# davidsd/sdpb

Hardware: AMD Instinct MI355X
Metric: interior-point iterations/sec at --precision 512 (higher is better)
Workload: dtype mw576 (fixed-width multi-word float, 18x32-bit limbs; Q syrk: exact integer product of a fixed-point image with 509 fraction bits)

## Files before the change

sdpb_amd/csrc/kernels.hpp:

```cpp
#pragma once
#include "dev.hpp"
#include "mw_wave.hpp"
#include "tiledot.hpp"

#include <algorithm>
#include <cmath>
#include <cstdlib>

namespace sdpb
{
using mw::Mw;
using mw::Acc;
constexpr int WG = 256;

template <int NL> MW_HD Mw<NL> mat_ld(const Batch &b, const MatDesc &d, int i, int j)
{
  return mw::load<NL>(b.p, (size_t)d.off + (size_t)i + (size_t)j * (size_t)d.ld);
}
template <int NL> MW_HD void mat_st(const Batch &b, const MatDesc &d, int i, int j, const Mw<NL> &v)
{
  mw::store<NL>(b.p, (size_t)d.off + (size_t)i + (size_t)j * (size_t)d.ld, v);
}

template <int NL, int STRIDE> MW_HD Mw<NL> smem_ld(const uint32_t *s, int idx)
// ... 1380 lines not shown
__global__ void __launch_bounds__(WG) k_dual_residues(Batch AY, mw::CPtr c, mw::Ptr d, const BlockDesc *blk)
{
  const int j = blockIdx.y;
  const BlockDesc bl = blk[j];
  const int p = blockIdx.x * WG + threadIdx.x;
  if(p >= bl.P)
    return;
  int cb, rb, k;
  decode_p(p, bl.K, cb, rb, k);
  Mw<NL> acc = mw::load<NL>(c, (size_t)bl.voff + p);
  for(int b = 0; b < 2; ++b)
    {
      const MatDesc dy = AY.d[2 * j + b];
      acc = mw::sub(acc, mat_ld<NL>(AY, dy, cb * bl.K + k, rb * bl.K + k));
    }
  mw::store<NL>(d, (size_t)bl.voff + p, acc);
}

template <int NL> __global__ void __launch_bounds__(WG) k_scale_bases(Batch bases, mw::CPtr a, Batch scaled, const BlockDesc *blk)
{
  const int q = blockIdx.y;
  const BlockDesc bl = blk[q >> 1];
  const MatDesc dbs = bases.d[q], dsc = scaled.d[q];
  const int rs = bl.rows[q & 1], K = bl.K;
  const int idx = blockIdx.x * WG + threadIdx.x;
  if(idx >= dsc.rows * dsc.cols)
    return;
  const int k = idx % K, col = idx / K, pair = col / rs, jj = col % rs;
  mat_st<NL>(scaled, dsc, k, col, mw::mul(mat_ld<NL>(bases, dbs, jj, k), mw::load<NL>(a, (size_t)bl.voff + (size_t)pair * K + k)));
}
template <int NL>
__global__ void __launch_bounds__(WG) k_constraint_weighted_sum(Batch bases, Batch scaled, Batch out, Batch addend,
                                                                int addend_sign, const BlockDesc *blk)
{
  const int q = blockIdx.y;
  const BlockDesc bl = blk[q >> 1];
  const MatDesc dout = out.d[q], dbs = bases.d[q], dsc = scaled.d[q];
  const int n = dout.rows, rs = bl.rows[q & 1];
  const int idx = blockIdx.x * WG + threadIdx.x;
  if(idx >= n * n)
    return;
  const int I = idx % n, Jc = idx / n;
  const int bi = I / rs, i = I % rs, bj = Jc / rs, jj = Jc % rs;
  const int hi = bi > bj ? bi : bj, lo = bi > bj ? bj : bi;
  const int col = (hi * (hi + 1) / 2 + lo) * rs + jj;
  Acc<NL> sum = mw::acc_zero<NL>();
  for(int k = 0; k < bl.K; ++k)
    mw::acc_fma(sum, mat_ld<NL>(bases, dbs, i, k), mat_ld<NL>(scaled, dsc, k, col));
  Mw<NL> acc = mw::acc_result(sum);
  if(hi != lo)
    acc = mw::mul_2exp(acc, -1);
  if(addend_sign)
    {
      const Mw<NL> ad = mat_ld<NL>(addend, addend.d[q], I, Jc);
      acc = addend_sign > 0 ? mw::add(acc, ad) : mw::sub(acc, ad);
    }
  mat_st<NL>(out, dout, I, Jc, acc);
}

template <int NL>
__global__ void __launch_bounds__(WG)
  k_schur_rhs2(Batch basesT, Batch Z, mw::CPtr dres, mw::Ptr dx, const BlockDesc *blk)
{
  const int j = blockIdx.y, t = threadIdx.x;
  const BlockDesc bl = blk[j];
  const int pair = blockIdx.x;
  if(pair >= bl.m * (bl.m + 1) / 2)
    return;
  int cb = 0;
  while((cb + 1) * (cb + 2) / 2 <= pair)
    ++cb;
  const int rb = pair - cb * (cb + 1) / 2;
  const int K = bl.K, KL = K < WG ? K : WG, G = WG / KL;
  const int kk = t % KL, g = t / KL;
  __shared__ Mw<NL> part[WG];
  for(int k0 = 0; k0 < K; k0 += KL)
    {
      const int k = k0 + kk;
      Acc<NL> colsum = mw::acc_zero<NL>();
      if(g < G && k < K)
        for(int b = 0; b < 2; ++b)
          {
            const int rs = bl.rows[b];
            const MatDesc dz = Z.d[2 * j + b], dbt = basesT.d[2 * j + b];
            for(int i = g; i < rs; i += G)
              {
                Acc<NL> zq = mw::acc_zero<NL>();
                for(int l = 0; l < rs; ++l)
                  mw::acc_fma(zq, mat_ld<NL>(Z, dz, cb * rs + l, rb * rs + i), mat_ld<NL>(basesT, dbt, k, l));
                mw::acc_fma(colsum, mw::acc_result(zq), mat_ld<NL>(basesT, dbt, k, i));
              }
          }
      part[t] = mw::acc_result(colsum);
      __syncthreads();
      if(g == 0 && k < K)
        {
          const size_t p = (size_t)bl.voff + (size_t)pair * K + k;
          Acc<NL> sum = mw::acc_zero<NL>();
          mw::acc_add(sum, mw::load<NL>(dres, p), 1u);
          for(int gg = 0; gg < G; ++gg)
            mw::acc_add(sum, part[gg * KL + kk], 1u);
          mw::store<NL>(dx, p, mw::acc_result(sum));
        }
      __syncthreads();
    }
}

template <int NL, bool TRANS>
__global__ void __launch_bounds__(WG) k_vec_trsm(Batch L, Batch Li, Batch X)
{
  const int q = blockIdx.x, t = threadIdx.x;
  const MatDesc dl = L.d[q], di = Li.d[q], dx = X.d[q];
  const int n = dl.rows;
  if(n == 0)
    return;
  constexpr int SEG = WG / PB;
  const int i = t % PB, seg = t / PB;
  const int panels = (n + PB - 1) / PB;
  __shared__ Mw<NL> sx[PB], part[WG];
  auto vec = [&](int r) { return (size_t)dx.off + (size_t)r * dx.ld; };
  for(int pp = 0; pp < panels; ++pp)
    {
      const int p = TRANS ? panels - 1 - pp : pp;
      const int k0 = p * PB, nb = n - k0 < PB ? n - k0 : PB;
      Acc<NL> acc = mw::acc_zero<NL>();
      if(i < nb)
        {
          const int lo = TRANS ? k0 + nb : 0, hi = TRANS ? n : k0;
          for(int k = lo + seg; k < hi; k += SEG)
            {
              const Mw<NL> l = TRANS ? mat_ld<NL>(L, dl, k, k0 + i) : mat_ld<NL>(L, dl, k0 + i, k);
              mw::acc_fms(acc, l, mw::load<NL>(X.p, vec(k)));
            }
          if(seg == 0)
            mw::acc_add(acc, mw::load<NL>(X.p, vec(k0 + i)));
        }
      part[t] = mw::acc_result(acc);
      __syncthreads();
      if(t < nb)
        {
          Acc<NL> s = mw::acc_zero<NL>();
          for(int gsg = 0; gsg < SEG; ++gsg)
            mw::acc_add(s, part[gsg * PB + t]);
          sx[t] = mw::acc_result(s);
        }
      __syncthreads();
      acc = mw::acc_zero<NL>();
      if(i < nb)
        for(int k = seg; k < nb; k += SEG)
          if(TRANS ? k >= i : k <= i)
            mw::acc_fma(acc, TRANS ? mat_ld<NL>(Li, di, k0 + k, k0 + i) : mat_ld<NL>(Li, di, k0 + i, k0 + k), sx[k]);
      part[t] = mw::acc_result(acc);
      __syncthreads();
      if(t < nb)
        {
          Acc<NL> s = mw::acc_zero<NL>();
          for(int gsg = 0; gsg < SEG; ++gsg)
            mw::acc_add(s, part[gsg * PB + t]);
          mw::store<NL>(X.p, vec(k0 + t), mw::acc_result(s));
        }
      __syncthreads();
    }
}

template <int NL, bool SQUARE>
__global__ void __launch_bounds__(WG) k_gemv_t_partial(Batch MT, mw::CPtr v, mw::Ptr part, const BlockDesc *blk, int N)
{
  const int j = blockIdx.y;
  const BlockDesc bl = blk[j];
  const int n = blockIdx.x * WG + threadIdx.x;
  if(n >= N)
    return;
  const MatDesc dm = MT.d[j];
  Acc<NL> acc = mw::acc_zero<NL>();
  for(int p = 0; p < bl.P; ++p)
    {
      const Mw<NL> a = mat_ld<NL>(MT, dm, n, p);
      if(SQUARE)
        mw::acc_fma(acc, a, a);
      else
        mw::acc_fma(acc, a, mw::load<NL>(v, (size_t)bl.voff + p));
    }
  mw::store<NL>(part, (size_t)j * N + n, mw::acc_result(acc));
}
template <int NL>
__global__ void __launch_bounds__(WG) k_sum_partials(mw::CPtr part, int J, int N, mw::CPtr base, int has_base, int sign, mw::Ptr out)
{
  constexpr int SP_G = 8, SP_N = WG / SP_G;
  const int i = threadIdx.x % SP_N, g = threadIdx.x / SP_N;
  const int n = blockIdx.x * SP_N + i;
  __shared__ Mw<NL> sm[WG];
  Acc<NL> acc = mw::acc_zero<NL>();
  if(n < N)
    for(int j = g; j < J; j += SP_G)
      mw::acc_add(acc, mw::load<NL>(part, (size_t)j * N + n), sign < 0 ? 1u : 0u);
  sm[threadIdx.x] = mw::acc_result(acc);
  __syncthreads();
  if(g != 0 || n >= N)
    return;
  Acc<NL> tot = mw::acc_zero<NL>();
  for(int gg = 0; gg < SP_G; ++gg)
    mw::acc_add(tot, sm[gg * SP_N + i]);
  if(has_base)
    mw::acc_add(tot, mw::load<NL>(base, n));
  mw::store<NL>(out, n, mw::acc_result(tot));
}
constexpr int SP_ROWS = WG / 8;
template <int NL>
__global__ void __launch_bounds__(WG) k_gemv_n(Batch MT, mw::CPtr v, mw::Ptr out, const BlockDesc *blk, int N, int sign)
{
  const int j = blockIdx.y;
  const BlockDesc bl = blk[j];
  const int lane = threadIdx.x & 63, sub = threadIdx.x >> 6;
  const int p = blockIdx.x * 4 + sub;
  Acc<NL> sum = mw::acc_zero<NL>();
  if(p < bl.P)
    {
      const MatDesc dm = MT.d[j];
      for(int n = lane; n < N; n += 64)
        mw::acc_fma(sum, mat_ld<NL>(MT, dm, n, p), mw::load<NL>(v, n));
    }
#if defined(__HIP_DEVICE_COMPILE__)
  {
    const Mw<NL> mine = mw::acc_result(sum);
    Acc<NL> a = mw::acc_zero<NL>();
    for(int g = 0; g < 8; ++g)
      mw::acc_add(a, wave_get<NL>(mine, g * 8 + (lane & 7)));
    const Mw<NL> s8 = mw::acc_result(a);
    Acc<NL> t = mw::acc_zero<NL>();
    if(p < bl.P)
      mw::acc_add(t, mw::load<NL>(out, (size_t)bl.voff + p));
    for(int g = 0; g < 8; ++g)
      mw::acc_add(t, wave_get<NL>(s8, g), sign < 0 ? 1u : 0u);
    if(lane == 0 && p < bl.P)
      mw::store<NL>(out, (size_t)bl.voff + p, mw::acc_result(t));
  }
#else
  __shared__ uint32_t sm[(NL + 2) * WG];
  smem_st<NL, WG>(sm, threadIdx.x, mw::acc_result(sum));
  __syncthreads();
  if(lane < 8)
    {
      Acc<NL> a = mw::acc_zero<NL>();
      for(int g = 0; g < 8; ++g)
        mw::acc_add(a, smem_ld<NL, WG>(sm, sub * 64 + g * 8 + lane));
      smem_st<NL, WG>(sm, threadIdx.x, mw::acc_result(a));
    }
  __syncthreads();
  if(lane == 0 && p < bl.P)
    {
      Acc<NL> a = mw::acc_zero<NL>();
      mw::acc_add(a, mw::load<NL>(out, (size_t)bl.voff + p));
      for(int g = 0; g < 8; ++g)
        mw::acc_add(a, smem_ld<NL, WG>(sm, sub * 64 + g), sign < 0 ? 1u : 0u);
      mw::store<NL>(out, (size_t)bl.voff + p, mw::acc_result(a));
    }
#endif
}

template <int FX> constexpr bool fx_two_level()
{
#ifdef SDPB_SYRK_ONE_LEVEL
  return false;
#else
  return FX % 4 == 0 && FX <= 32;
#endif
}
template <int NL> constexpr int fx_limbs() { return (NL - 2 >= 14 && (NL - 2) % 4 != 0) ? ((NL - 2 + 3) / 4) * 4 : NL - 2; }
#ifndef SDPB_TOOM4_MAX_FX
#define SDPB_TOOM4_MAX_FX 48
#endif
template <int FX> constexpr bool fx_toom4()
{
#if defined(SDPB_SYRK_ONE_LEVEL) || defined(SDPB_SYRK_NO_TOOM4)
  return false;
#else
  return FX % 4 == 0 && FX >= 16 && FX <= SDPB_TOOM4_MAX_FX;
#endif
}
template <int FX> constexpr bool fx_toom4k()
{
#if defined(SDPB_SYRK_NO_TOOM4K)
  return false;
#else
  return fx_toom4<FX>() && (FX == 16 || FX == 24 || FX == 32);
#endif
}
template <int FX> constexpr bool fx_toom5k()
{
#if defined(SDPB_SYRK_NO_TOOM5K)
  return false;
#else
  return fx_toom4k<FX>() && FX == 16;
#endif
}
constexpr int T5_LB = 28;
constexpr uint32_t T5_MASK = (1u << T5_LB) - 1u;
constexpr int T5_H = 55;
template <int FX> constexpr int fx_nprod() { return fx_toom5k<FX>() ? 27 : 21; }
template <int FX> constexpr int fx_part_limbs() { return fx_toom5k<FX>() ? 5 : 2 * (FX / 8) + 1; }
template <int FX> constexpr int toom_wb() { return fx_toom5k<FX>() ? 102 : 32 * (FX / 4) - (fx_toom4k<FX>() ? 6 : 4); }
template <int FX> constexpr int fx_planes()
{
  return fx_toom5k<FX>() ? 27 * 2 : fx_toom4k<FX>() ? 21 * (FX / 8) : fx_toom4<FX>() ? 7 * (FX / 4) : fx_two_level<FX>() ? 9 * (FX / 4) : 3 * (FX / 2);
}
template <int FX> constexpr int fx_frac_bits()
{
  return fx_toom5k<FX>() ? 5 * toom_wb<FX>() - 1 : fx_toom4<FX>() ? 4 * toom_wb<FX>() - 1 : fx_two_level<FX>() ? 32 * FX - 7 : 32 * FX - 3;
}
template <int FX> constexpr int fx_col_slot(int c) { return fx_toom5k<FX>() ? 32 * (c / 32) + 2 * (c % 16) + (c % 32) / 16 : c; }
template <int FX> constexpr size_t fx_row_slots(size_t cols) { return fx_toom5k<FX>() ? (cols + 31) / 32 * 32 : cols; }
template <int FX> MW_HD size_t fx_elem(size_t idx, int N)
{
  if constexpr(fx_toom5k<FX>())
    return idx / (size_t)N * fx_row_slots<FX>((size_t)N) + (size_t)fx_col_slot<FX>((int)(idx % (size_t)N));
  else
    return idx;
}
template <int FX> constexpr size_t fx_image_stride(size_t rows, size_t cols, int rb)
{
  return fx_toom4k<FX>() ? (rows + rb - 1) / rb * rb * fx_row_slots<FX>(cols) + 64 : rows * cols;
}
template <int FX> constexpr int syrk_tile_edge() { return fx_toom4k<FX>() ? 32 : 16; }

template <int BIT0, int NB, int W, int OUT> MW_HD void bits_slice(const uint32_t (&x)[W], uint32_t (&out)[OUT])
{
  constexpr int q = BIT0 / 32, r = BIT0 % 32;
#pragma unroll
  for(int i = 0; i < OUT; ++i)
    {
      const uint32_t lo = (q + i < W) ? x[q + i < W ? q + i : 0] : 0u;
      const uint32_t hi = (q + i + 1 < W) ? x[q + i + 1 < W ? q + i + 1 : 0] : 0u;
      uint32_t v = r ? ((lo >> r) | (hi << ((32 - r) & 31))) : lo;
      const int left = NB - 32 * i;
      if(left <= 0)
        v = 0;
      else if(left < 32)
        v &= (1u << (left & 31)) - 1u;
      out[i] = v;
    }
}

template <int W, int A> MW_HD void add_shifted(uint32_t (&w)[W], const uint32_t (&x)[A], int sh, bool negate)
{
  const int q = sh >> 5, r = sh & 31;
  uint64_t cy = negate ? 1u : 0u;
  const uint32_t mask = negate ? 0xffffffffu : 0u;
#pragma unroll
  for(int k = 0; k < W; ++k)
    {
      const int i0 = k - q;
      uint32_t lo = 0, hi = 0;
#pragma unroll
      for(int t = 0; t < A; ++t)
        {
          lo = (t == i0 - 1) ? x[t] : lo;
          hi = (t == i0) ? x[t] : hi;
        }
      const uint32_t limb = r ? ((hi << r) | (lo >> (32 - r))) : hi;
      const uint64_t s = (uint64_t)w[k] + (uint64_t)(limb ^ mask) + cy;
      w[k] = (uint32_t)s;
      cy = s >> 32;
    }
}

template <int FX> MW_HD void fx_store2(const uint32_t (&mag)[FX], bool negative, uint32_t *fx, size_t fx_stride, size_t idx);
template <int FX> MW_HD void fx_store4(const uint32_t (&mag)[FX], bool negative, uint32_t *fx, size_t fx_stride, size_t idx);
template <int FX> MW_HD void fx_store5(const uint32_t (&mag)[FX], bool negative, uint32_t *fx, size_t fx_stride, size_t idx);
template <int FX> MW_HD void fx_store(const uint32_t (&mag)[FX], bool negative, uint32_t *fx, size_t fx_stride, size_t idx)
{
  constexpr int M = FX / 2;
  static_assert(FX % 2 == 0 && FX >= 4, "FX = NL - 2 is even");
  if constexpr(fx_toom5k<FX>())
    {
      fx_store5<FX>(mag, negative, fx, fx_stride, idx);
      return;
    }
  else if constexpr(fx_toom4<FX>())
    {
      fx_store4<FX>(mag, negative, fx, fx_stride, idx);
      return;
    }
  else if constexpr(fx_two_level<FX>())
    {
      fx_store2<FX>(mag, negative, fx, fx_stride, idx);
      return;
    }
  uint32_t a[FX];
  uint64_t borrow = 0;
#pragma unroll
  for(int i = 0; i < FX; ++i)
    {
      const uint32_t c = (i == FX - 1) ? (1u << 29) : 0u;
      if(negative)
        {
          const uint64_t d = (uint64_t)c - (uint64_t)mag[i] - borrow;
          a[i] = (uint32_t)d;
          borrow = (d >> 63) & 1u;
        }
      else
        a[i] = mag[i] | c;
    }
  uint32_t lo[M], hi[M];
#pragma unroll
  for(int i = 0; i < M; ++i)
    {
      lo[i] = (i == M - 1) ? (a[i] & 0x7fffffffu) : a[i];
      const uint32_t up = (M + i < FX) ? a[M + i < FX ? M + i : 0] : 0u;
      hi[i] = (a[M - 1 + i] >> 31) | (up << 1);
    }
  uint64_t cy = 0;
#pragma unroll
  for(int i = 0; i < M; ++i)
    {
      const uint64_t s = (uint64_t)lo[i] + hi[i] + cy;
      cy = s >> 32;
      fx[(size_t)i * fx_stride + idx] = lo[i];
      fx[(size_t)(M + i) * fx_stride + idx] = hi[i];
      fx[(size_t)(2 * M + i) * fx_stride + idx] = (uint32_t)s;
    }
}

template <int FX> MW_HD void fx_store2(const uint32_t (&mag)[FX], bool negative, uint32_t *fx, size_t fx_stride, size_t idx)
{
  constexpr int M = FX / 2, M2 = FX / 4, FB = fx_frac_bits<FX>();
  static_assert(FB / 32 == FX - 1, "the bias bit sits in the top limb");
  uint32_t a[FX];
  uint64_t borrow = 0;
#pragma unroll
  for(int i = 0; i < FX; ++i)
    {
      const uint32_t c = (i == FX - 1) ? (1u << (FB % 32)) : 0u;
      if(negative)
        {
          const uint64_t d = (uint64_t)c - (uint64_t)mag[i] - borrow;
          a[i] = (uint32_t)d;
          borrow = (d >> 63) & 1u;
        }
      else
        a[i] = mag[i] | c;
    }
  uint32_t x[3][M];
  bits_slice<0, 32 * M - 3>(a, x[0]);
  bits_slice<32 * M - 3, 32 * M - 3>(a, x[1]);
  {
    uint64_t cy = 0;
#pragma unroll
    for(int i = 0; i < M; ++i)
      {
        const uint64_t t = (uint64_t)x[0][i] + x[1][i] + cy;
        x[2][i] = (uint32_t)t;
        cy = t >> 32;
      }
  }
#pragma unroll
  for(int k = 0; k < 3; ++k)
    {
      uint32_t p0[M2], p1[M2];
      bits_slice<0, 32 * M2 - 1>(x[k], p0);
      bits_slice<32 * M2 - 1, 32 * M2 - 1>(x[k], p1);
      uint32_t *o0 = fx + ((size_t)(3 * k) * fx_stride + idx) * M2, *o1 = fx + ((size_t)(3 * k + 1) * fx_stride + idx) * M2,
               *ot = fx + ((size_t)(3 * k + 2) * fx_stride + idx) * M2;
      uint64_t cy = 0;
#pragma unroll
      for(int i = 0; i < M2; ++i)
        {
          const uint64_t t = (uint64_t)p0[i] + p1[i] + cy;
          cy = t >> 32;
          o0[i] = p0[i];
          o1[i] = p1[i];
          ot[i] = (uint32_t)t;
        }
    }
}

struct alignas(16) PieceQuad
{
  uint32_t w[4];
};
struct alignas(8) PiecePair
{
  uint32_t w[2];
};
template <int M2> MW_HD void piece_load(const uint32_t *p, uint32_t (&x)[M2])
{
  if constexpr(M2 % 4 == 0)
    {
#pragma unroll
      for(int q = 0; q < M2 / 4; ++q)
        {
          const PieceQuad v = *reinterpret_cast<const PieceQuad *>(p + 4 * q);
#pragma unroll
          for(int l = 0; l < 4; ++l)
            x[4 * q + l] = v.w[l];
        }
    }
  else if constexpr(M2 % 2 == 0)
    {
#pragma unroll
      for(int q = 0; q < M2 / 2; ++q)
        {
          const PiecePair v = *reinterpret_cast<const PiecePair *>(p + 2 * q);
          x[2 * q] = v.w[0];
          x[2 * q + 1] = v.w[1];
        }
    }
  else
    {
#pragma unroll
      for(int l = 0; l < M2; ++l)
        x[l] = p[l];
    }
}
template <int M2> MW_HD void piece_store(uint32_t *p, const uint32_t (&x)[M2])
{
  if constexpr(M2 % 4 == 0)
    {
#pragma unroll
      for(int q = 0; q < M2 / 4; ++q)
        {
          PieceQuad v;
#pragma unroll
          for(int l = 0; l < 4; ++l)
            v.w[l] = x[4 * q + l];
          *reinterpret_cast<PieceQuad *>(p + 4 * q) = v;
        }
    }
  else if constexpr(M2 % 2 == 0)
    {
#pragma unroll
      for(int q = 0; q < M2 / 2; ++q)
        {
          PiecePair v;
          v.w[0] = x[2 * q];
          v.w[1] = x[2 * q + 1];
          *reinterpret_cast<PiecePair *>(p + 2 * q) = v;
        }
    }
  else
    {
#pragma unroll
      for(int l = 0; l < M2; ++l)
        p[l] = x[l];
    }
}

template <int A> MW_HD void sub_limbs(uint32_t (&d)[A], const uint32_t (&x)[A])
{
  uint64_t bw = 0;
#pragma unroll
  for(int k = 0; k < A; ++k)
    {
      const uint64_t t = (uint64_t)d[k] - (uint64_t)x[k] - bw;
      d[k] = (uint32_t)t;
      bw = (t >> 63) & 1u;
    }
}

template <int ML> MW_HD void toom5_lin(uint32_t (&out)[ML], const uint32_t (&p)[5][ML], uint32_t c0, uint32_t c1, uint32_t c2, uint32_t c3, uint32_t c4)
{
  uint64_t cy = 0;
#pragma unroll
  for(int i = 0; i < ML; ++i)
    {
      const uint64_t t = (uint64_t)p[0][i] * c0 + (uint64_t)p[1][i] * c1 + (uint64_t)p[2][i] * c2 + (uint64_t)p[3][i] * c3 + (uint64_t)p[4][i] * c4 + cy;
      out[i] = (uint32_t)t;
      cy = t >> 32;
    }
}
template <int POS, int NB, int ML> MW_HD uint32_t toom5_bits(const uint32_t (&x)[ML])
{
  constexpr int q = POS / 32, r = POS % 32;
  const uint32_t lo = q < ML ? x[q < ML ? q : 0] : 0u, hi = q + 1 < ML ? x[q + 1 < ML ? q + 1 : 0] : 0u;
  const uint32_t v = r ? ((lo >> r) | (hi << (32 - r))) : lo;
  return NB < 32 ? (v & ((1u << (NB < 32 ? NB : 0)) - 1u)) : v;
}
template <int FX> MW_HD void fx_store5(const uint32_t (&mag)[FX], bool negative, uint32_t *fx, size_t fx_stride, size_t idx)
{
  constexpr int WB = toom_wb<FX>(), FB = fx_frac_bits<FX>(), ML = (WB + 7 + 31) / 32, H = T5_H, LB = T5_LB;
  constexpr int TOPBIT = WB - 32 * (ML - 1);
  static_assert(FB == 5 * WB - 1 && FB / 32 == FX - 1, "a' = v + 2^FB fills five pieces of WB bits");
  static_assert(TOPBIT >= 0 && TOPBIT + 7 <= 32 && WB + 7 <= 2 * H && H + 1 <= 2 * LB, "121 b fits, the halves fit two limbs");
  uint32_t a[FX];
  uint64_t borrow = 0;
#pragma unroll
  for(int i = 0; i < FX; ++i)
    {
      const uint32_t c = (i == FX - 1) ? (1u << (FB % 32)) : 0u;
      if(negative)
        {
          const uint64_t d = (uint64_t)c - (uint64_t)mag[i] - borrow;
          a[i] = (uint32_t)d;
          borrow = (d >> 63) & 1u;
        }
      else
        a[i] = mag[i] | c;
    }
  uint32_t p[5][ML];
  bits_slice<0, WB>(a, p[0]);
  bits_slice<WB, WB>(a, p[1]);
  bits_slice<2 * WB, WB>(a, p[2]);
  bits_slice<3 * WB, WB>(a, p[3]);
  bits_slice<4 * WB, WB>(a, p[4]);
  uint32_t e[9][ML];
#pragma unroll
  for(int i = 0; i < ML; ++i)
    {
      e[0][i] = p[0][i];
      e[8][i] = p[4][i];
    }
  toom5_lin<ML>(e[1], p, 1, 1, 1, 1, 1);
  toom5_lin<ML>(e[3], p, 1, 2, 4, 8, 16);
  toom5_lin<ML>(e[5], p, 16, 8, 4, 2, 1);
  toom5_lin<ML>(e[7], p, 1, 3, 9, 27, 81);
  {
    uint32_t pos[ML], neg[ML];
    auto diff = [&](uint32_t (&out)[ML], uint32_t bias) {
      pos[ML - 1] += bias << TOPBIT;
      uint64_t bw = 0;
#pragma unroll
      for(int i = 0; i < ML; ++i)
        {
          const uint64_t t = (uint64_t)pos[i] - (uint64_t)neg[i] - bw;
          out[i] = (uint32_t)t;
          bw = (t >> 63) & 1u;
        }
    };
    toom5_lin<ML>(pos, p, 1, 0, 1, 0, 1);
    toom5_lin<ML>(neg, p, 0, 1, 0, 1, 0);
    diff(e[2], 2u);
    toom5_lin<ML>(pos, p, 1, 0, 4, 0, 16);
    toom5_lin<ML>(neg, p, 0, 2, 0, 8, 0);
    diff(e[4], 10u);
    toom5_lin<ML>(pos, p, 16, 0, 4, 0, 1);
    toom5_lin<ML>(neg, p, 0, 8, 0, 2, 0);
    diff(e[6], 10u);
  }
#pragma unroll
  for(int g = 0; g < 9; ++g)
    {
      uint32_t lo[2], hi[2], mid[2];
      lo[0] = toom5_bits<0, LB>(e[g]);
      lo[1] = toom5_bits<LB, H - LB>(e[g]);
      hi[0] = toom5_bits<H, LB>(e[g]);
      hi[1] = toom5_bits<H + LB, H - LB>(e[g]);
      const uint32_t s0 = lo[0] + hi[0];
      mid[0] = s0 & T5_MASK;
      mid[1] = lo[1] + hi[1] + (s0 >> LB);
      piece_store<2>(fx + ((size_t)(3 * g + 0) * fx_stride + idx) * 2, lo);
      piece_store<2>(fx + ((size_t)(3 * g + 1) * fx_stride + idx) * 2, hi);
      piece_store<2>(fx + ((size_t)(3 * g + 2) * fx_stride + idx) * 2, mid);
    }
}

template <int M2> MW_HD void toom_lin(uint32_t (&out)[M2], const uint32_t (&p)[4][M2], uint32_t c0, uint32_t c1, uint32_t c2, uint32_t c3)
{
  uint64_t cy = 0;
#pragma unroll
  for(int i = 0; i < M2; ++i)
    {
      const uint64_t t = (uint64_t)p[0][i] * c0 + (uint64_t)p[1][i] * c1 + (uint64_t)p[2][i] * c2 + (uint64_t)p[3][i] * c3 + cy;
      out[i] = (uint32_t)t;
      cy = t >> 32;
    }
}
template <int FX> MW_HD void fx_store4(const uint32_t (&mag)[FX], bool negative, uint32_t *fx, size_t fx_stride, size_t idx)
{
  constexpr int M2 = FX / 4, WB = toom_wb<FX>(), FB = fx_frac_bits<FX>();
  constexpr int TOPBIT = WB - 32 * (M2 - 1);
  static_assert(FB == 4 * WB - 1 && FB / 32 == FX - 1, "a' = v + 2^FB fills four pieces of WB bits");
  static_assert(TOPBIT >= 0 && TOPBIT + 4 <= 32, "15 b fits the top limb");
  uint32_t a[FX];
  uint64_t borrow = 0;
#pragma unroll
  for(int i = 0; i < FX; ++i)
    {
      const uint32_t c = (i == FX - 1) ? (1u << (FB % 32)) : 0u;
      if(negative)
        {
          const uint64_t d = (uint64_t)c - (uint64_t)mag[i] - borrow;
          a[i] = (uint32_t)d;
          borrow = (d >> 63) & 1u;
        }
      else
        a[i] = mag[i] | c;
    }
  uint32_t p[4][M2];
  bits_slice<0, WB>(a, p[0]);
  bits_slice<WB, WB>(a, p[1]);
  bits_slice<2 * WB, WB>(a, p[2]);
  bits_slice<3 * WB, WB>(a, p[3]);
  uint32_t e[7][M2];
#pragma unroll
  for(int i = 0; i < M2; ++i)
    {
      e[0][i] = p[0][i];
      e[6][i] = p[3][i];
    }
  toom_lin<M2>(e[1], p, 1, 1, 1, 1);
  toom_lin<M2>(e[3], p, 1, 2, 4, 8);
  toom_lin<M2>(e[5], p, 8, 4, 2, 1);
  {
    uint32_t pos[M2], neg[M2];
    toom_lin<M2>(pos, p, 1, 0, 1, 0);
    toom_lin<M2>(neg, p, 0, 1, 0, 1);
    pos[M2 - 1] += 2u << TOPBIT;
    uint64_t bw = 0;
#pragma unroll
    for(int i = 0; i < M2; ++i)
      {
        const uint64_t t = (uint64_t)pos[i] - (uint64_t)neg[i] - bw;
        e[2][i] = (uint32_t)t;
        bw = (t >> 63) & 1u;
      }
    toom_lin<M2>(pos, p, 1, 0, 4, 0);
    toom_lin<M2>(neg, p, 0, 2, 0, 8);
    pos[M2 - 1] += 10u << TOPBIT;
    bw = 0;
#pragma unroll
    for(int i = 0; i < M2; ++i)
      {
        const uint64_t t = (uint64_t)pos[i] - (uint64_t)neg[i] - bw;
        e[4][i] = (uint32_t)t;
        bw = (t >> 63) & 1u;
      }
  }
  if constexpr(fx_toom4k<FX>())
    {
      constexpr int M3 = FX / 8, H = 16 * M2 - 1;
#pragma unroll
      for(int g = 0; g < 7; ++g)
        {
          uint32_t lo[M3], hi[M3], mid[M3];
          bits_slice<0, H>(e[g], lo);
          bits_slice<H, H>(e[g], hi);
          uint64_t cy = 0;
#pragma unroll
          for(int i = 0; i < M3; ++i)
            {
              const uint64_t t = (uint64_t)lo[i] + hi[i] + cy;
              mid[i] = (uint32_t)t;
              cy = t >> 32;
            }
          piece_store<M3>(fx + ((size_t)(3 * g + 0) * fx_stride + idx) * M3, lo);
          piece_store<M3>(fx + ((size_t)(3 * g + 1) * fx_stride + idx) * M3, hi);
          piece_store<M3>(fx + ((size_t)(3 * g + 2) * fx_stride + idx) * M3, mid);
        }
    }
  else
    {
#pragma unroll
      for(int g = 0; g < 7; ++g)
        {
          uint32_t *o = fx + ((size_t)g * fx_stride + idx) * M2;
#pragma unroll
          for(int i = 0; i < M2; ++i)
            o[i] = e[g][i];
        }
    }
}
template <int FX> MW_HD void toom_piece_load(const uint32_t *fx, size_t fx_stride, int g, size_t e, uint32_t (&x)[FX / 4])
{
  constexpr int M2 = FX / 4;
  if constexpr(fx_toom4k<FX>())
    {
      constexpr int M3 = FX / 8, H = 16 * M2 - 1;
      uint32_t lo[M2], lo3[M3], hi[M3];
      piece_load<M3>(fx + ((size_t)(3 * g + 0) * fx_stride + e) * M3, lo3);
      piece_load<M3>(fx + ((size_t)(3 * g + 1) * fx_stride + e) * M3, hi);
#pragma unroll
      for(int i = 0; i < M2; ++i)
        lo[i] = i < M3 ? lo3[i < M3 ? i : 0] : 0u;
      add_shifted<M2, M3>(lo, hi, H, false);
#pragma unroll
      for(int i = 0; i < M2; ++i)
        x[i] = lo[i];
    }
  else
    {
      const uint32_t *src = fx + ((size_t)g * fx_stride + e) * M2;
#pragma unroll
      for(int i = 0; i < M2; ++i)
        x[i] = src[i];
    }
}
template <int Z> MW_HD void z_add(uint32_t (&d)[Z], const uint32_t (&x)[Z])
{
  uint64_t cy = 0;
#pragma unroll
  for(int k = 0; k < Z; ++k)
    {
      const uint64_t t = (uint64_t)d[k] + x[k] + cy;
      d[k] = (uint32_t)t;
      cy = t >> 32;
    }
}
template <int Z> MW_HD void z_sub(uint32_t (&d)[Z], const uint32_t (&x)[Z])
{
  uint64_t bw = 0;
#pragma unroll
  for(int k = 0; k < Z; ++k)
    {
      const uint64_t t = (uint64_t)d[k] - (uint64_t)x[k] - bw;
      d[k] = (uint32_t)t;
      bw = (t >> 63) & 1u;
    }
}
template <int Z> MW_HD void z_addmul(uint32_t (&d)[Z], const uint32_t (&x)[Z], uint32_t c, bool subtract)
{
  uint32_t t[Z];
  uint64_t cy = 0;
#pragma unroll
  for(int k = 0; k < Z; ++k)
    {
      const uint64_t u = (uint64_t)x[k] * c + cy;
      t[k] = (uint32_t)u;
      cy = u >> 32;
    }
  if(subtract)
    z_sub<Z>(d, t);
  else
    z_add<Z>(d, t);
}
template <int Z> MW_HD void z_sar(uint32_t (&d)[Z], int bits)
{
  const uint32_t fill = 0u - (d[Z - 1] >> 31);
#pragma unroll
  for(int k = 0; k < Z; ++k)
    {
      const uint32_t up = k + 1 < Z ? d[k + 1 < Z ? k + 1 : 0] : fill;
      d[k] = (d[k] >> bits) | (up << (32 - bits));
    }
}
template <int Z> MW_HD void z_shl(uint32_t (&d)[Z], int sh)
{
  const int q = sh >> 5, r = sh & 31;
  uint32_t t[Z];
#pragma unroll
  for(int k = 0; k < Z; ++k)
    {
      uint32_t lo = 0, hi = 0;
#pragma unroll
      for(int u = 0; u < Z; ++u)
        {
          hi = (u == k - q) ? d[u] : hi;
          lo = (u == k - q - 1) ? d[u] : lo;
        }
      t[k] = r ? ((hi << r) | (lo >> (32 - r))) : hi;
    }
#pragma unroll
  for(int k = 0; k < Z; ++k)
    d[k] = t[k];
}
template <int Z> MW_HD void z_divexact(uint32_t (&d)[Z], uint32_t c, uint32_t cinv)
{
  uint32_t carry = 0;
#pragma unroll
  for(int k = 0; k < Z; ++k)
    {
      const uint32_t b = d[k] < carry ? 1u : 0u;
      const uint32_t q = (d[k] - carry) * cinv;
      d[k] = q;
      carry = (uint32_t)(((uint64_t)q * c) >> 32) + b;
    }
}
template <int Z> MW_HD void toom4_interpolate(uint32_t (&w)[7][Z])
{
  z_add<Z>(w[5], w[4]);
  {
    uint32_t t[Z];
#pragma unroll
    for(int k = 0; k < Z; ++k)
      t[k] = w[4][k];
    z_sub<Z>(t, w[1]);
    z_sar<Z>(t, 1);
#pragma unroll
    for(int k = 0; k < Z; ++k)
      w[1][k] = t[k];
  }
  z_sub<Z>(w[4], w[0]);
  z_sub<Z>(w[4], w[1]);
  z_sar<Z>(w[4], 2);
  z_addmul<Z>(w[4], w[6], 16, true);
  {
    uint32_t t[Z];
#pragma unroll
    for(int k = 0; k < Z; ++k)
      t[k] = w[2][k];
    z_sub<Z>(t, w[3]);
    z_sar<Z>(t, 1);
#pragma unroll
    for(int k = 0; k < Z; ++k)
      w[3][k] = t[k];
  }
  z_sub<Z>(w[2], w[3]);
  z_addmul<Z>(w[5], w[2], 65, true);
  z_sub<Z>(w[2], w[6]);
  z_sub<Z>(w[2], w[0]);
  z_addmul<Z>(w[5], w[2], 45, false);
  z_sar<Z>(w[5], 1);
  z_sub<Z>(w[4], w[2]);
  z_divexact<Z>(w[4], 3, 0xAAAAAAABu);
  z_sub<Z>(w[2], w[4]);
  {
    uint32_t t[Z];
#pragma unroll
    for(int k = 0; k < Z; ++k)
      t[k] = w[5][k];
    z_sub<Z>(t, w[1]);
#pragma unroll
    for(int k = 0; k < Z; ++k)
      w[1][k] = t[k];
  }
  z_addmul<Z>(w[5], w[3], 8, true);
  z_divexact<Z>(w[5], 9, 0x38E38E39u);
  z_sub<Z>(w[3], w[5]);
  z_divexact<Z>(w[1], 15, 0xEEEEEEEFu);
  z_add<Z>(w[1], w[5]);
  z_sar<Z>(w[1], 1);
  z_sub<Z>(w[5], w[1]);
}

template <int NL, int FX>
__global__ void __launch_bounds__(WG) k_normalize_fx(mw::CPtr PT, size_t count, int N, mw::CPtr inv_norm, uint32_t *fx, size_t fx_stride)
{
  constexpr int FB = fx_frac_bits<FX>();
  for(size_t idx = (size_t)blockIdx.x * WG + threadIdx.x; idx < count; idx += (size_t)gridDim.x * WG)
    {
      const Mw<NL> t = mw::mul(mw::load<NL>(PT, idx), mw::load<NL>(inv_norm, idx % N));
      uint32_t w[NL];
      bool sat = false;
      if(mw::is_zero(t))
        {
#pragma unroll
          for(int i = 0; i < NL; ++i)
            w[i] = 0;
        }
      else
        {
#pragma unroll
          for(int i = 0; i < NL; ++i)
            w[i] = t.m[i];
          const int s = 32 * NL - FB - t.e;
          if(t.e >= 1)
            sat = true;
          else if(s >= 32 * NL)
            {
#pragma unroll
              for(int i = 0; i < NL; ++i)
                w[i] = 0;
            }
          else
            {
              mw::shr_limbs<NL>(w, (uint32_t)s >> 5);
// ... 548 lines not shown
  {
    uint32_t m[Z];
#pragma unroll
    for(int k = 0; k < Z; ++k)
      m[k] = 0;
    z_addmul<Z>(m, t, 10, false);
    z_shl<Z>(m, WB);
#pragma unroll
    for(int k = 0; k < Z; ++k)
      t[k] = 0;
    z_addmul<Z>(t, n, 50, false);
    z_shl<Z>(t, 2 * WB);
    z_add<Z>(t, m);
  }
#pragma unroll
  for(int k = 0; k < Z; ++k)
    toomU[(size_t)(Z + k) * N + col] = t[k];
}
template <int FX>
__global__ void __launch_bounds__(WG)
  k_syrk4_finish(const uint32_t *part, int nsplit, size_t part_stride, const uint32_t *tile_list, size_t total, const uint32_t *toomU,
                 uint32_t *acc, size_t acc_stride, int N, int col0, int col1)
{
  constexpr int M2 = FX / 4, A2 = 2 * M2 + 1, Z = 2 * M2 + 2, W = 2 * FX + 2, WB = toom_wb<FX>();
  const size_t pidx = (size_t)blockIdx.x * WG + threadIdx.x;
  int i, j;
  if(pidx >= total || !syrk_packed_decode<syrk_tile_edge<FX>()>(pidx, tile_list, N, col0, col1, i, j))
    return;
  const size_t idx = (size_t)i + (size_t)j * N;
  uint32_t w[7][Z];
  constexpr int GRP[7] = {0, 4, 1, 2, 3, 5, 6};
  if constexpr(fx_toom4k<FX>())
    {
      constexpr int M3 = FX / 8, A3 = 2 * M3 + 1, H = 16 * M2 - 1;
#pragma unroll
      for(int q = 0; q < 7; ++q)
        {
          uint32_t g3[3][A3];
#pragma unroll
          for(int u = 0; u < 3; ++u)
            {
              uint64_t cy = 0;
#pragma unroll
              for(int k = 0; k < A3; ++k)
                {
                  for(int s = 0; s < nsplit; ++s)
                    cy += part[(((size_t)s * 21 + 3 * GRP[q] + u) * A3 + k) * part_stride + pidx];
                  g3[u][k] = (uint32_t)cy;
                  cy >>= 32;
                }
            }
          sub_limbs<A3>(g3[2], g3[0]);
          sub_limbs<A3>(g3[2], g3[1]);
#pragma unroll
          for(int k = 0; k < Z; ++k)
            w[q][k] = k < A3 ? g3[0][k < A3 ? k : 0] : 0u;
          add_shifted<Z, A3>(w[q], g3[2], H, false);
          add_shifted<Z, A3>(w[q], g3[1], 2 * H, false);
        }
    }
  else
    {
#pragma unroll
  for(int q = 0; q < 7; ++q)
    {
      uint64_t cy = 0;
#pragma unroll
      for(int k = 0; k < Z; ++k)
        {
          if(k < A2)
            for(int s = 0; s < nsplit; ++s)
              cy += part[(((size_t)s * 7 + GRP[q]) * A2 + k) * part_stride + pidx];
          w[q][k] = (uint32_t)cy;
          cy >>= 32;
        }
    }
    }
  {
    uint32_t u[Z];
#pragma unroll
    for(int k = 0; k < Z; ++k)
      u[k] = toomU[(size_t)k * N + i];
    z_sub<Z>(w[3], u);
#pragma unroll
    for(int k = 0; k < Z; ++k)
      u[k] = toomU[(size_t)k * N + j];
    z_sub<Z>(w[3], u);
#pragma unroll
    for(int k = 0; k < Z; ++k)
      u[k] = toomU[(size_t)(Z + k) * N + i];
    z_sub<Z>(w[1], u);
#pragma unroll
    for(int k = 0; k < Z; ++k)
      u[k] = toomU[(size_t)(Z + k) * N + j];
    z_sub<Z>(w[1], u);
  }
  toom4_interpolate<Z>(w);
  uint32_t g[W];
#pragma unroll
  for(int k = 0; k < W; ++k)
    g[k] = k < Z ? w[0][k < Z ? k : 0] : 0u;
#pragma unroll
  for(int q = 1; q < 7; ++q)
    add_shifted<W, Z>(g, w[q], q * WB, false);
#pragma unroll
  for(int k = 0; k < W; ++k)
    acc[(size_t)k * acc_stride + idx] = g[k];
}


#ifndef SDPB_SYRK2_UNROLL
#define SDPB_SYRK2_UNROLL 4
#endif
template <int FX, int RBG, bool TOOM = false>
__global__ void __launch_bounds__(WG, SDPB_SYRK_WAVES)
  k_syrk_fx2(const uint32_t *__restrict__ fx_in, size_t fx_stride, unsigned nrows, int N, uint32_t *acc, size_t acc_stride,
             const uint32_t *tile_list, int ntile, int nsplit, unsigned rows_per_split, const uint32_t *zero_piece, int packed)
{
  constexpr int M2 = FX / 4, M = FX / 2, A2 = 2 * M2 + 1, A = 2 * M + 2, W = 2 * FX + 2;
  constexpr int NP = RBG * 16, GL = NP / WG;
  static_assert(NP % WG == 0, "a pass stages a whole number of pieces per lane");
  const uint32_t *fx = (const uint32_t *)__builtin_assume_aligned(fx_in, 16);
  const int nitem = ntile * nsplit, per = (nitem + 7) / 8;
  const int item = (int)(blockIdx.x % 8) * per + (int)(blockIdx.x / 8);
  if((int)(blockIdx.x / 8) >= per || item >= nitem)
    return;
  const int split = item / ntile, tile = item % ntile;
  const unsigned row_begin = (unsigned)split * rows_per_split;
  const unsigned row_end = (row_begin + rows_per_split < nrows && split + 1 < nsplit) ? row_begin + rows_per_split : nrows;
  acc += (size_t)split * (TOOM ? 7 * A2 : W) * acc_stride;
  const uint32_t tt = tile_list[tile];
  const int ti = (int)(tt >> 16), tj = (int)(tt & 0xffffu);
  const int li = threadIdx.x & 15, lj = threadIdx.x >> 4;
  const int i = ti * 16 + li, j = tj * 16 + lj;
  __shared__ __attribute__((aligned(16))) uint32_t sa[2 * NP * M2];
  __shared__ __attribute__((aligned(16))) uint32_t sb[2 * NP * M2];
  constexpr int NGRP = TOOM ? 7 : 9;
  constexpr int NG = TOOM ? (FX > 32 ? 4 : 7) : FX >= 32 ? 3 : 9, SWEEPS = (NGRP + NG - 1) / NG;
  uint32_t g2[NG][A2];
  uint32_t x[TOOM ? 1 : 3][TOOM ? 1 : A];
#if defined(__HIP_DEVICE_COMPILE__)
  constexpr bool DIRECT = (M2 == 4);
#else
  constexpr bool DIRECT = false;
#endif
  uint32_t va[DIRECT ? 1 : GL][M2], vb[DIRECT ? 1 : GL][M2];
  auto fetch = [&](int g, unsigned r0, int into) __attribute__((always_inline)) {
#pragma unroll
    for(int t = 0; t < GL; ++t)
      {
        const int e = threadIdx.x + t * WG;
        const int col = e & 15, rr = e >> 4;
        const unsigned r = r0 + rr;
        const int ca = ti * 16 + col, cb = tj * 16 + col;
        const bool ok = r < row_end;
        const uint32_t *row = fx + ((size_t)g * fx_stride + (size_t)(ok ? r : row_begin) * (size_t)N) * M2;
        if constexpr(DIRECT)
          {
#if defined(__HIP_DEVICE_COMPILE__)
            const uint32_t *pa = (ok && ca < N) ? row + (size_t)ca * M2 : zero_piece;
            const uint32_t *pb = (ok && cb < N) ? row + (size_t)cb * M2 : zero_piece;
            const int wbase = (into * NP + t * WG + (int)(threadIdx.x & ~63u)) * M2;
            __builtin_amdgcn_global_load_lds((const __attribute__((address_space(1))) void *)pa,
                                             (__attribute__((address_space(3))) void *)(sa + wbase), 16, 0, 0);
            __builtin_amdgcn_global_load_lds((const __attribute__((address_space(1))) void *)pb,
                                             (__attribute__((address_space(3))) void *)(sb + wbase), 16, 0, 0);
#endif
          }
        else
          {
            piece_load<M2>(row + (size_t)(ca < N ? ca : 0) * M2, va[t]);
            piece_load<M2>(row + (size_t)(cb < N ? cb : 0) * M2, vb[t]);
            const uint32_t ma = (ok && ca < N) ? 0xffffffffu : 0u, mb = (ok && cb < N) ? 0xffffffffu : 0u;
#pragma unroll
            for(int l = 0; l < M2; ++l)
              {
                va[t][l] &= ma;
                vb[t][l] &= mb;
              }
          }
      }
  };
  auto store = [&](int buf) __attribute__((always_inline)) {
    if constexpr(!DIRECT)
      {
#pragma unroll
        for(int t = 0; t < GL; ++t)
          {
            const int e = threadIdx.x + t * WG;
            piece_store<M2>(sa + (buf * NP + e) * M2, va[t]);
            piece_store<M2>(sb + (buf * NP + e) * M2, vb[t]);
          }
      }
  };
  auto second_level = [&](int k, int g0) __attribute__((always_inline)) {
    if constexpr(TOOM)
      return;
    else
      {
    sub_limbs<A2>(g2[g0 + 2], g2[g0]);
    sub_limbs<A2>(g2[g0 + 2], g2[g0 + 1]);
#pragma unroll
    for(int q = 0; q < A; ++q)
      x[k][q] = q < A2 ? g2[g0][q < A2 ? q : 0] : 0u;
    add_shifted<A, A2>(x[k], g2[g0 + 2], 32 * M2 - 1, false);
    add_shifted<A, A2>(x[k], g2[g0 + 1], 64 * M2 - 2, false);
      }
  };
#pragma unroll
  for(int sweep = 0; sweep < SWEEPS; ++sweep)
  {
#pragma unroll
  for(int g = 0; g < NG; ++g)
#pragma unroll
    for(int k = 0; k < A2; ++k)
      g2[g][k] = 0;
  if(sweep > 0)
    __syncthreads();
  const int ngs = NGRP - sweep * NG < NG ? NGRP - sweep * NG : NG;
  fetch(sweep * NG, row_begin, 0);
  store(0);
  __syncthreads();
  int buf = 0;
  for(unsigned r0 = row_begin; r0 < row_end; r0 += RBG)
    {
#pragma unroll
      for(int g = 0; g < NG; ++g)
        {
          if(g >= ngs)
            continue;
          fetch(sweep * NG + (g < ngs - 1 ? g + 1 : 0), g < ngs - 1 ? r0 : r0 + RBG, buf ^ 1);
          uint64_t c[2 * M2 - 1];
          uint32_t h[2 * M2 - 1];
#pragma unroll
          for(int k = 0; k < 2 * M2 - 1; ++k)
            {
              c[k] = 0;
              h[k] = 0;
            }
          const uint32_t *pa = sa + (buf * NP + li) * M2, *pb = sb + (buf * NP + lj) * M2;
#pragma unroll SDPB_SYRK2_UNROLL
          for(int rr = 0; rr < RBG; ++rr)
            {
              uint32_t a[M2], b[M2];
              piece_load<M2>(pa + rr * 16 * M2, a);
              piece_load<M2>(pb + rr * 16 * M2, b);
              SyrkColumns<M2, 0>::run(a, b, c, h);
            }
          syrk_fold<M2, A2>(g2[g], c, h);
          store(buf ^ 1);
          __syncthreads();
          buf ^= 1;
        }
    }
  if constexpr(TOOM)
    {
      if(i < N && j <= i)
        {
          const size_t o = (size_t)tile * 256 + threadIdx.x;
#pragma unroll
          for(int g = 0; g < NG; ++g)
            if(g < ngs)
              {
#pragma unroll
                for(int k = 0; k < A2; ++k)
                  acc[(size_t)((sweep * NG + g) * A2 + k) * acc_stride + o] = g2[g][k];
              }
        }
    }
  else if constexpr(SWEEPS == 3)
    second_level(sweep, 0);
  }
  if constexpr(TOOM)
    return;
  else
  {
  if constexpr(SWEEPS == 1)
    {
#pragma unroll
      for(int k = 0; k < 3; ++k)
        second_level(k, 3 * k);
    }
  if(i < N && j <= i)
    {
      sub_limbs<A>(x[2], x[0]);
      sub_limbs<A>(x[2], x[1]);
      uint32_t w[W];
#pragma unroll
      for(int k = 0; k < W; ++k)
        w[k] = k < A ? x[0][k < A ? k : 0] : 0u;
      add_shifted<W, A>(w, x[2], 32 * M - 3, false);
      add_shifted<W, A>(w, x[1], 64 * M - 6, false);
      const size_t o = packed ? (size_t)tile * 256 + threadIdx.x : (size_t)i + (size_t)j * N;
#pragma unroll
      for(int k = 0; k < W; ++k)
        acc[(size_t)k * acc_stride + o] = w[k];
    }
  }
}

#ifndef SDPB_SYRK3_WAVES
#define SDPB_SYRK3_WAVES 3
#endif
#ifndef SDPB_SYRK3_LAZY_TRIP
#define SDPB_SYRK3_LAZY_TRIP 32
#endif
template <int FX, int RBG>
__global__ void __launch_bounds__(WG, SDPB_SYRK3_WAVES)
  k_syrk_fx3(const uint32_t *__restrict__ fx_in, size_t fx_stride, unsigned nrows, int N, uint32_t *acc, size_t acc_stride,
             const uint32_t *tile_list, int ntile, int nsplit, unsigned rows_per_split, int gsplit)
{
  constexpr bool LAZY = fx_toom5k<FX>();
  constexpr int M3 = FX / 8, A3 = fx_part_limbs<FX>(), NPROD = fx_nprod<FX>();
  static_assert(M3 >= 2 && M3 <= 4 && (!LAZY || (M3 == 2 && RBG <= 32)), "accumulators of 2 x 2 outputs in registers; 2 x 32 rows between carries");
  constexpr int ROWW = 32 * M3, UPR = ROWW / 4, NPAIR = RBG * UPR, GL = NPAIR / WG;
  static_assert(NPAIR % WG == 0, "a pass stages a whole number of units per lane");
  const uint32_t *fx = (const uint32_t *)__builtin_assume_aligned(fx_in, 4);
  const int nitem = ntile * nsplit * gsplit, per = (nitem + 7) / 8;
  const int item = (int)(blockIdx.x % 8) * per + (int)(blockIdx.x / 8);
  if((int)(blockIdx.x / 8) >= per || item >= nitem)
    return;
  const int sg = item / ntile, tile = item % ntile, split = sg / gsplit;
  const int prod_begin = (sg % gsplit) * (NPROD / gsplit), prod_end = prod_begin + NPROD / gsplit;
  const unsigned row_begin = (unsigned)split * rows_per_split;
  const unsigned row_end = (row_begin + rows_per_split < nrows && split + 1 < nsplit) ? row_begin + rows_per_split : nrows;
  acc += (size_t)split * NPROD * A3 * acc_stride;
  const uint32_t tt = tile_list[tile];
  const int ti = (int)(tt >> 16), tj = (int)(tt & 0xffffu);
  const int li = threadIdx.x & 15, lj = threadIdx.x >> 4;
  const int i0 = ti * 32 + li, j0 = tj * 32 + lj;
  const bool half_i = ti * 32 + 16 < N, half_j = tj * 32 + 16 < N;
  const int mask = 1 | (half_i ? 2 : 0) | ((half_j && tj < ti) ? 4 : 0) | ((half_i && half_j) ? 8 : 0);
  __shared__ __attribute__((aligned(16))) uint32_t sa[2 * NPAIR * 4 + 64];
  __shared__ __attribute__((aligned(16))) uint32_t sb[2 * NPAIR * 4 + 64];
  uint64_t cc[4][2 * M3 - 1];
  uint32_t hh[4][2 * M3 - 1];
  uint64_t dd[4][2 * M3 - 1];
#if defined(__HIP_DEVICE_COMPILE__)
  constexpr bool DIRECT = true;
#else
  constexpr bool DIRECT = false;
#endif
  const size_t NS = fx_row_slots<FX>((size_t)N);
  uint32_t va[DIRECT ? 1 : GL][4], vb[DIRECT ? 1 : GL][4];
  uint32_t offa[GL], offb[GL];
#pragma unroll
  for(int t = 0; t < GL; ++t)
    {
      const int e = threadIdx.x + t * WG;
      const int unit = e % UPR, rr = e / UPR;
      offa[t] = (uint32_t)(((size_t)rr * NS + ti * 32) * M3 + 4 * unit);
      offb[t] = (uint32_t)(((size_t)rr * NS + tj * 32) * M3 + 4 * unit);
    }
  auto fetch = [&](int g, unsigned r0, int into) __attribute__((always_inline)) {
    const uint32_t *base = fx + ((size_t)g * fx_stride + (size_t)r0 * NS) * M3;
#pragma unroll
    for(int t = 0; t < GL; ++t)
      {
        if constexpr(DIRECT)
          {
#if defined(__HIP_DEVICE_COMPILE__)
            const int wbase = (into * NPAIR + t * WG + (int)(threadIdx.x & ~63u)) * 4;
            __builtin_amdgcn_global_load_lds((const __attribute__((address_space(1))) void *)(base + offa[t]),
                                             (__attribute__((address_space(3))) void *)(sa + wbase), 16, 0, 0);
            __builtin_amdgcn_global_load_lds((const __attribute__((address_space(1))) void *)(base + offb[t]),
                                             (__attribute__((address_space(3))) void *)(sb + wbase), 16, 0, 0);
#endif
          }
        else
          {
#pragma unroll
            for(int l = 0; l < 4; ++l)
              {
                va[t][l] = base[offa[t] + l];
                vb[t][l] = base[offb[t] + l];
              }
          }
      }
  };
  auto store = [&](int buf) __attribute__((always_inline)) {
    if constexpr(!DIRECT)
      {
#pragma unroll
        for(int t = 0; t < GL; ++t)
          {
            const int e = threadIdx.x + t * WG;
            piece_store<4>(sa + (buf * NPAIR + e) * 4, va[t]);
            piece_store<4>(sb + (buf * NPAIR + e) * 4, vb[t]);
          }
      }
  };
  auto rows = [&](auto mask_c, int buf, uint64_t (&c)[4][2 * M3 - 1], uint32_t (&h)[4][2 * M3 - 1]) __attribute__((always_inline)) {
    constexpr int MASK = decltype(mask_c)::value;
#if defined(__HIP_DEVICE_COMPILE__)
    constexpr bool ASM_ROWS = (M3 == 2);
#else
    constexpr bool ASM_ROWS = false;
#endif
    if constexpr(ASM_ROWS)
      {
#if defined(__HIP_DEVICE_COMPILE__)
    typedef uint32_t u32x4 __attribute__((ext_vector_type(4)));
    constexpr int LSTEP = LAZY ? 2 * M3 : M3;
    const uint32_t la = (uint32_t)(uintptr_t)(__attribute__((address_space(3))) uint32_t *)(sa + buf * NPAIR * 4 + li * LSTEP);
    const uint32_t lb = (uint32_t)(uintptr_t)(__attribute__((address_space(3))) uint32_t *)(sb + buf * NPAIR * 4 + lj * LSTEP);
    static_assert(RBG % 4 == 0 && M3 == 2, "four rows per trip, offsets in units of 8 bytes");
#define FX3_P(C, H, X, Y) "v_mad_u64_u32 %" #C ", vcc, %" #X ", %" #Y ", %" #C "\n\tv_addc_co_u32 %" #H ", vcc, 0, %" #H ", vcc\n\t"
#define FX3_L(C, X, Y) "v_mad_u64_u32 %" #C ", vcc, %" #X ", %" #Y ", %" #C "\n\t"
#define FX3_MAC_BOTH(o0, o1, a0x, a0y, a1x, a1y, bx, by)                                                                                   \
  asm volatile(FX3_P(0, 6, 12, 16) FX3_P(3, 9, 14, 16) FX3_P(1, 7, 12, 17) FX3_P(4, 10, 14, 17) FX3_P(1, 7, 13, 16) FX3_P(4, 10, 15, 16)   \
                 FX3_P(2, 8, 13, 17) FX3_P(5, 11, 15, 17)                                                                                  \
               : "+v"(c[o0][0]), "+v"(c[o0][1]), "+v"(c[o0][2]), "+v"(c[o1][0]), "+v"(c[o1][1]), "+v"(c[o1][2]), "+v"(h[o0][0]),           \
                 "+v"(h[o0][1]), "+v"(h[o0][2]), "+v"(h[o1][0]), "+v"(h[o1][1]), "+v"(h[o1][2])                                            \
               : "v"(a0x), "v"(a0y), "v"(a1x), "v"(a1y), "v"(bx), "v"(by)                                                                  \
               : "vcc")
#define FX3_MAC_ONE(o0, ax, ay, bx, by)                                                                                                    \
  asm volatile(FX3_P(0, 3, 6, 8) FX3_P(1, 4, 6, 9) FX3_P(1, 4, 7, 8) FX3_P(2, 5, 7, 9)                                                     \
               : "+v"(c[o0][0]), "+v"(c[o0][1]), "+v"(c[o0][2]), "+v"(h[o0][0]), "+v"(h[o0][1]), "+v"(h[o0][2])                            \
               : "v"(ax), "v"(ay), "v"(bx), "v"(by)                                                                                        \
               : "vcc")
#define FX3L_MAC_BOTH(o0, o1, a0x, a0y, a1x, a1y, bx, by)                                                                                  \
  asm volatile(FX3_L(0, 6, 10) FX3_L(3, 8, 10) FX3_L(1, 6, 11) FX3_L(4, 8, 11) FX3_L(1, 7, 10) FX3_L(4, 9, 10) FX3_L(2, 7, 11)             \
                 FX3_L(5, 9, 11)                                                                                                           \
               : "+v"(c[o0][0]), "+v"(c[o0][1]), "+v"(c[o0][2]), "+v"(c[o1][0]), "+v"(c[o1][1]), "+v"(c[o1][2])                            \
               : "v"(a0x), "v"(a0y), "v"(a1x), "v"(a1y), "v"(bx), "v"(by)                                                                  \
               : "vcc")
#define FX3L_MAC_ONE(o0, ax, ay, bx, by)                                                                                                   \
  asm volatile(FX3_L(0, 3, 5) FX3_L(1, 3, 6) FX3_L(1, 4, 5) FX3_L(2, 4, 6)                                                                 \
               : "+v"(c[o0][0]), "+v"(c[o0][1]), "+v"(c[o0][2])                                                                            \
               : "v"(ax), "v"(ay), "v"(bx), "v"(by)                                                                                        \
               : "vcc")
#define FX3_QUADRANTS(BOTH, ONE, va, vb)                                                                                                   \
  if constexpr(MASK == 15)                                                                                                                 \
    {                                                                                                                                      \
      BOTH(0, 1, va.x, va.y, va.z, va.w, vb.x, vb.y);                                                                                      \
      BOTH(2, 3, va.x, va.y, va.z, va.w, vb.z, vb.w);                                                                                      \
    }                                                                                                                                      \
  else if constexpr(MASK == 11)                                                                                                            \
    {                                                                                                                                      \
      BOTH(0, 1, va.x, va.y, va.z, va.w, vb.x, vb.y);                                                                                      \
      ONE(3, va.z, va.w, vb.z, vb.w);                                                                                                      \
    }                                                                                                                                      \
  else if constexpr(MASK == 5)                                                                                                             \
    {                                                                                                                                      \
      ONE(0, va.x, va.y, vb.x, vb.y);                                                                                                      \
      ONE(2, va.x, va.y, vb.z, vb.w);                                                                                                      \
    }                                                                                                                                      \
  else                                                                                                                                     \
    ONE(0, va.x, va.y, vb.x, vb.y);
#define FX3_MACS(va, vb) FX3_QUADRANTS(FX3_MAC_BOTH, FX3_MAC_ONE, va, vb)
#define FX3L_MACS(va, vb) FX3_QUADRANTS(FX3L_MAC_BOTH, FX3L_MAC_ONE, va, vb)
#define FX3_NEXT(wa, wb, ra, rb, O0, O1)                                                                                                   \
  asm volatile("s_waitcnt lgkmcnt(0)\n\tds_read2_b64 %2, %4 offset0:" #O0 " offset1:" #O1 "\n\tds_read2_b64 %3, %5 offset0:" #O0            \
               " offset1:" #O1                                                                                                             \
               : "+v"(wa), "+v"(wb), "=&v"(ra), "=&v"(rb)                                                                                  \
               : "v"(xa), "v"(xb)                                                                                                          \
               : "memory")
#define FX3L_NEXT(wa, wb, ra, rb, ROW)                                                                                                     \
  asm volatile("s_waitcnt lgkmcnt(0)\n\tds_read_b128 %2, %4 offset:%6\n\tds_read_b128 %3, %5 offset:%6"                                   \
               : "+v"(wa), "+v"(wb), "=&v"(ra), "=&v"(rb)                                                                                  \
               : "v"(xa), "v"(xb), "n"((ROW) * 256)                                                                                        \
               : "memory")
#define FX3L_ROWS2(R)                                                                                                                      \
  FX3L_NEXT(a0, b0, a1, b1, (R) + 1);                                                                                                      \
  FX3L_MACS(a0, b0)                                                                                                                        \
  FX3L_NEXT(a1, b1, a0, b0, (R) + 2);                                                                                                      \
  FX3L_MACS(a1, b1)
#define FX3L_ROWS8(R) FX3L_ROWS2(R) FX3L_ROWS2((R) + 2) FX3L_ROWS2((R) + 4) FX3L_ROWS2((R) + 6)
    u32x4 a0, b0, a1, b1;
    if constexpr(LAZY)
      {
        constexpr int TRIP = (RBG % SDPB_SYRK3_LAZY_TRIP == 0) ? SDPB_SYRK3_LAZY_TRIP : 8;
        static_assert(RBG % 8 == 0 && (TRIP == 8 || TRIP == 16 || TRIP == 32) && RBG * 256 < 65536, "whole trips, the offsets fit 16 bits");
        {
          const uint32_t xa = la, xb = lb;
          asm volatile("ds_read_b128 %0, %2\n\tds_read_b128 %1, %3" : "=&v"(a0), "=&v"(b0) : "v"(xa), "v"(xb) : "memory");
        }
#pragma unroll 1
        for(int rr = 0; rr < RBG; rr += TRIP)
          {
            const uint32_t xa = la + rr * 256, xb = lb + rr * 256;
            FX3L_ROWS8(0)
            if constexpr(TRIP >= 16)
              {
                FX3L_ROWS8(8)
              }
            if constexpr(TRIP >= 32)
              {
                FX3L_ROWS8(16)
                FX3L_ROWS8(24)
              }
          }
      }
    else
      {
        {
          const uint32_t xa = la, xb = lb;
          asm volatile("ds_read2_b64 %0, %2 offset0:0 offset1:16\n\tds_read2_b64 %1, %3 offset0:0 offset1:16" : "=&v"(a0), "=&v"(b0) : "v"(xa), "v"(xb) : "memory");
        }
#pragma unroll 1
        for(int rr = 0; rr < RBG; rr += 4)
          {
            const uint32_t xa = la + rr * 256, xb = lb + rr * 256;
            FX3_NEXT(a0, b0, a1, b1, 32, 48);
            FX3_MACS(a0, b0)
            FX3_NEXT(a1, b1, a0, b0, 64, 80);
            FX3_MACS(a1, b1)
            FX3_NEXT(a0, b0, a1, b1, 96, 112);
            FX3_MACS(a0, b0)
            FX3_NEXT(a1, b1, a0, b0, 128, 144);
            FX3_MACS(a1, b1)
          }
      }
    asm volatile("s_waitcnt lgkmcnt(0)" : "+v"(a0), "+v"(b0)::"memory");
#undef FX3L_ROWS8
#undef FX3L_ROWS2
#undef FX3L_NEXT
#undef FX3_NEXT
#undef FX3L_MACS
#undef FX3_MACS
#undef FX3_QUADRANTS
#undef FX3L_MAC_ONE
#undef FX3L_MAC_BOTH
#undef FX3_MAC_ONE
#undef FX3_MAC_BOTH
#undef FX3_P
#undef FX3_L
#endif
      }
    else
      {
        constexpr int LSTEP = LAZY ? 2 * M3 : M3, SECOND = LAZY ? M3 : 16 * M3;
        const uint32_t *pa = sa + buf * NPAIR * 4 + li * LSTEP, *pb = sb + buf * NPAIR * 4 + lj * LSTEP;
#pragma unroll SDPB_SYRK2_UNROLL
        for(int rr = 0; rr < RBG; ++rr)
          {
            uint32_t a0[M3], a1[M3], b0[M3], b1[M3];
            piece_load<M3>(pa + rr * ROWW, a0);
            piece_load<M3>(pb + rr * ROWW, b0);
            if constexpr((MASK & 10) != 0)
              piece_load<M3>(pa + rr * ROWW + SECOND, a1);
            if constexpr((MASK & 12) != 0)
              piece_load<M3>(pb + rr * ROWW + SECOND, b1);
            if constexpr(LAZY)
              {
                auto lazy = [&](const uint32_t (&x)[M3], const uint32_t (&y)[M3], uint64_t (&cs)[2 * M3 - 1]) {
                  cs[0] += (uint64_t)x[0] * y[0];
                  cs[1] += (uint64_t)x[0] * y[1] + (uint64_t)x[1] * y[0];
                  cs[2] += (uint64_t)x[1] * y[1];
                };
                lazy(a0, b0, c[0]);
                if constexpr((MASK & 2) != 0)
                  lazy(a1, b0, c[1]);
                if constexpr((MASK & 4) != 0)
                  lazy(a0, b1, c[2]);
                if constexpr((MASK & 8) != 0)
                  lazy(a1, b1, c[3]);
              }
            else
              {
            SyrkColumns<M3, 0>::run(a0, b0, c[0], h[0]);
            if constexpr((MASK & 2) != 0)
              SyrkColumns<M3, 0>::run(a1, b0, c[1], h[1]);
            if constexpr((MASK & 4) != 0)
              SyrkColumns<M3, 0>::run(a0, b1, c[2], h[2]);
            if constexpr((MASK & 8) != 0)
              SyrkColumns<M3, 0>::run(a1, b1, c[3], h[3]);
              }
          }
      }
  };
  for(int prod = prod_begin; prod < prod_end; ++prod)
    {
#pragma unroll
      for(int o = 0; o < 4; ++o)
#pragma unroll
        for(int k = 0; k < 2 * M3 - 1; ++k)
          {
            cc[o][k] = 0;
            hh[o][k] = 0;
          }
#pragma unroll
      for(int o = 0; o < 4; ++o)
#pragma unroll
        for(int k = 0; k < 2 * M3 - 1; ++k)
          dd[o][k] = 0;
      auto carry_columns = [&](bool all) __attribute__((always_inline)) {
        if constexpr(LAZY)
          {
#pragma unroll
            for(int o = 0; o < 4; ++o)
              {
                dd[o][1] += cc[o][1] >> 32;
                cc[o][1] &= 0xffffffffull;
              }
            if(all)
              {
#pragma unroll
                for(int o = 0; o < 4; ++o)
                  {
                    dd[o][0] += cc[o][0] >> 32;
                    cc[o][0] &= 0xffffffffull;
                    dd[o][2] += cc[o][2] >> 32;
                    cc[o][2] &= 0xffffffffull;
                  }
              }
          }
      };
      if(prod > prod_begin)
        __syncthreads();
      fetch(prod, row_begin, 0);
      store(0);
      __syncthreads();
      auto sweep = [&](auto mask_c) __attribute__((always_inline)) {
        int buf = 0;
        unsigned pass = 0;
        for(unsigned r0 = row_begin; r0 < row_end; r0 += RBG)
          {
            fetch(prod, r0 + RBG < row_end ? r0 + RBG : row_begin, buf ^ 1);
            rows(mask_c, buf, cc, hh);
            ++pass;
            if(LAZY && (pass & 1u) == 0)
              carry_columns((pass & 3u) == 0);
            store(buf ^ 1);
            __syncthreads();
            buf ^= 1;
          }
      };
      switch(mask)
        {
        case 15: sweep(std::integral_constant<int, 15>()); break;
        case 11: sweep(std::integral_constant<int, 11>()); break;
        case 5: sweep(std::integral_constant<int, 5>()); break;
        default: sweep(std::integral_constant<int, 1>()); break;
        }
#pragma unroll
      for(int o = 0; o < 4; ++o)
        {
          const int i = i0 + 16 * (o & 1), j = j0 + 16 * (o >> 1);
          if(!((mask >> o) & 1) || i >= N || j > i)
            continue;
          uint32_t g[A3];
#pragma unroll
          for(int k = 0; k < A3; ++k)
            g[k] = 0;
          if constexpr(LAZY)
            {
              unsigned __int128 v = 0;
#pragma unroll
              for(int k = 0; k < 2 * M3 - 1; ++k)
                v += ((unsigned __int128)cc[o][k] + ((unsigned __int128)dd[o][k] << 32)) << (T5_LB * k);
              g[0] = (uint32_t)v;
              g[1] = (uint32_t)(v >> 32);
              g[2] = (uint32_t)(v >> 64);
              g[3] = (uint32_t)(v >> 96);
            }
          else
          syrk_fold<M3, A3>(g, cc[o], hh[o]);
          const size_t at = (size_t)tile * 1024 + (size_t)(li + 16 * (o & 1)) + (size_t)(lj + 16 * (o >> 1)) * 32;
#pragma unroll
          for(int k = 0; k < A3; ++k)
            acc[(size_t)(prod * A3 + k) * acc_stride + at] = g[k];
        }
    }
}

template <int FX>
__global__ void __launch_bounds__(WG) k_syrk3_sum_splits(uint32_t *part, int nsplit, size_t part_stride, const uint32_t *tile_list, size_t total, int N,
                                                         int col0, int col1)
{
  constexpr int A3 = fx_part_limbs<FX>(), NPROD = fx_nprod<FX>();
  const size_t pidx = (size_t)blockIdx.x * WG + threadIdx.x;
  const int prod = blockIdx.y;
  int i, j;
  if(pidx >= total || !syrk_packed_decode<32>(pidx, tile_list, N, col0, col1, i, j))
    return;
  uint32_t out[A3];
  uint64_t cy = 0;
#pragma unroll
  for(int k = 0; k < A3; ++k)
    {
#pragma unroll 8
      for(int s = 0; s < nsplit; ++s)
        cy += part[(((size_t)s * NPROD + prod) * A3 + k) * part_stride + pidx];
      out[k] = (uint32_t)cy;
      cy >>= 32;
    }
#pragma unroll
  for(int k = 0; k < A3; ++k)
    part[((size_t)prod * A3 + k) * part_stride + pidx] = out[k];
}

constexpr uint32_t inv_mod_2_32(uint32_t c)
{
  uint32_t x = c;
  for(int i = 0; i < 5; ++i)
    x *= 2u - c * x;
  return x;
}
constexpr int T5_Z = 10;
MW_HD void toom5_value(const uint32_t *fx, size_t fx_stride, int point, size_t e, uint32_t (&w)[4])
{
  const PiecePair lo = *reinterpret_cast<const PiecePair *>(fx + ((size_t)(3 * point + 0) * fx_stride + e) * 2);
  const PiecePair hi = *reinterpret_cast<const PiecePair *>(fx + ((size_t)(3 * point + 1) * fx_stride + e) * 2);
  w[0] = lo.w[0] | (lo.w[1] << 28);
  w[1] = (lo.w[1] >> 4) | (hi.w[0] << 23);
  w[2] = (hi.w[0] >> 9) | (hi.w[1] << 19);
  w[3] = hi.w[1] >> 13;
}
template <int FX>
__global__ void __launch_bounds__(WG) k_fx_colsum5(const uint32_t *fx, size_t fx_stride, unsigned nrows, int N, unsigned rows_per_slice, uint32_t *partial)
{
  constexpr int A = 5, G = 5;
  const int lane = threadIdx.x & 63, col = blockIdx.x * 64 + lane, phase = threadIdx.x >> 6;
  const unsigned r_begin = blockIdx.y * rows_per_slice, r_end = (r_begin + rows_per_slice < nrows) ? r_begin + rows_per_slice : nrows;
  uint32_t sum[G][A];
#pragma unroll
  for(int u = 0; u < G; ++u)
#pragma unroll
    for(int k = 0; k < A; ++k)
      sum[u][k] = 0;
  if(col < N)
    for(unsigned r = r_begin + phase; r < r_end; r += 4)
      {
        const size_t e = (size_t)r * fx_row_slots<FX>((size_t)N) + (size_t)fx_col_slot<FX>(col);
#pragma unroll
        for(int u = 0; u < G; ++u)
          {
            const int point = u == 0 ? 0 : u == 1 ? 1 : u == 2 ? 3 : u == 3 ? 5 : 8;
            uint32_t src[4];
            toom5_value(fx, fx_stride, point, e, src);
            uint64_t cy = 0;
#pragma unroll
            for(int k = 0; k < A; ++k)
              {
                const uint64_t t = (uint64_t)sum[u][k] + (k < 4 ? src[k < 4 ? k : 0] : 0u) + cy;
                sum[u][k] = (uint32_t)t;
                cy = t >> 32;
              }
          }
      }
  __shared__ uint32_t sm[3 * G * A * 64];
  if(phase > 0)
    {
#pragma unroll
      for(int u = 0; u < G; ++u)
#pragma unroll
        for(int k = 0; k < A; ++k)
          sm[(((phase - 1) * G + u) * A + k) * 64 + lane] = sum[u][k];
    }
  __syncthreads();
  if(phase == 0 && col < N)
    {
      for(int p = 0; p < 3; ++p)
#pragma unroll
        for(int u = 0; u < G; ++u)
          {
            uint64_t cy = 0;
#pragma unroll
            for(int k = 0; k < A; ++k)
              {
                const uint64_t t = (uint64_t)sum[u][k] + sm[((p * G + u) * A + k) * 64 + lane] + cy;
                sum[u][k] = (uint32_t)t;
                cy = t >> 32;
              }
          }
#pragma unroll
      for(int u = 0; u < G; ++u)
#pragma unroll
        for(int k = 0; k < A; ++k)
          partial[(((size_t)blockIdx.y * G + u) * A + k) * N + col] = sum[u][k];
    }
}
template <int FX>
__global__ void __launch_bounds__(WG)
  k_fx_colsum5_final(const uint32_t *partial, int nslices, int N, uint32_t *acc, size_t acc_stride, uint32_t *toomU, unsigned long long nrows_local)
{
  constexpr int A = 5, G = 5, W = 2 * FX + 2, WB = toom_wb<FX>(), Z = T5_Z;
  const int col = blockIdx.x * WG + threadIdx.x;
  if(col >= N)
    return;
  uint32_t g[G][Z];
#pragma unroll
  for(int u = 0; u < G; ++u)
#pragma unroll
    for(int k = 0; k < Z; ++k)
      g[u][k] = 0;
  for(int sl = 0; sl < nslices; ++sl)
#pragma unroll
    for(int u = 0; u < G; ++u)
      {
        uint64_t cy = 0;
#pragma unroll
        for(int k = 0; k < A + 1; ++k)
          {
            const uint64_t t = (uint64_t)g[u][k] + (k < A ? partial[(((size_t)sl * G + u) * A + (k < A ? k : 0)) * N + col] : 0u) + cy;
            g[u][k] = (uint32_t)t;
            cy = t >> 32;
          }
      }
  uint32_t s[5][Z], u[Z], v[Z], t[Z];
#pragma unroll
  for(int k = 0; k < Z; ++k)
    {
      s[0][k] = g[0][k];
      s[4][k] = g[4][k];
      u[k] = g[1][k];
      v[k] = g[2][k];
      t[k] = g[3][k];
    }
  z_sub<Z>(u, s[0]);
  z_sub<Z>(u, s[4]);
  z_sub<Z>(v, s[0]);
  z_addmul<Z>(v, s[4], 16, true);
  z_addmul<Z>(t, s[0], 16, true);
  z_sub<Z>(t, s[4]);
#pragma unroll
  for(int k = 0; k < Z; ++k)
    s[2][k] = 0;
  z_addmul<Z>(s[2], u, 10, false);
  z_sub<Z>(s[2], v);
  z_sub<Z>(s[2], t);
  z_sar<Z>(s[2], 1);
  z_sub<Z>(v, t);
  z_sar<Z>(v, 1);
  z_divexact<Z>(v, 3u, inv_mod_2_32(3u));
  z_sub<Z>(u, s[2]);
#pragma unroll
  for(int k = 0; k < Z; ++k)
    {
      s[3][k] = u[k];
      s[1][k] = u[k];
    }
  z_add<Z>(s[3], v);
  z_sar<Z>(s[3], 1);
  z_sub<Z>(s[1], v);
  z_sar<Z>(s[1], 1);
  {
    uint32_t w[W];
#pragma unroll
    for(int k = 0; k < W; ++k)
      w[k] = k < Z ? s[0][k < Z ? k : 0] : 0u;
#pragma unroll
    for(int q = 1; q < 5; ++q)
      add_shifted<W, Z>(w, s[q], q * WB, false);
#pragma unroll
    for(int k = 0; k < W; ++k)
      acc[(size_t)k * acc_stride + (size_t)N * N + col] = w[k];
  }
  uint32_t n[Z];
#pragma unroll
  for(int k = 0; k < Z; ++k)
    n[k] = k == 0 ? (uint32_t)nrows_local : k == 1 ? (uint32_t)(nrows_local >> 32) : 0u;
  auto emit = [&](int which, uint32_t c0, bool n0, uint32_t c1, bool n1, uint32_t c2, bool n2, uint32_t c3, bool n3, uint32_t c4, bool n4, bool ten) {
    uint32_t e[Z], m[Z];
#pragma unroll
    for(int k = 0; k < Z; ++k)
      e[k] = m[k] = 0;
    z_addmul<Z>(e, s[0], c0, n0);
    z_addmul<Z>(e, s[1], c1, n1);
    z_addmul<Z>(e, s[2], c2, n2);
    z_addmul<Z>(e, s[3], c3, n3);
    z_addmul<Z>(e, s[4], c4, n4);
    if(ten)
      {
#pragma unroll
        for(int k = 0; k < Z; ++k)
          t[k] = 0;
        z_addmul<Z>(t, e, 10, false);
        z_shl<Z>(t, WB);
        z_addmul<Z>(m, n, 50, false);
        z_shl<Z>(m, 2 * WB);
      }
    else
      {
#pragma unroll
        for(int k = 0; k < Z; ++k)
          {
            t[k] = e[k];
            m[k] = n[k];
          }
        z_shl<Z>(t, WB + 1);
        z_shl<Z>(m, 2 * WB + 1);
      }
    z_add<Z>(t, m);
#pragma unroll
    for(int k = 0; k < Z; ++k)
      toomU[(size_t)(which * Z + k) * N + col] = t[k];
  };
  emit(0, 1, false, 1, true, 1, false, 1, true, 1, false, false);
  emit(1, 1, false, 2, true, 4, false, 8, true, 16, false, true);
  emit(2, 16, false, 8, true, 4, false, 2, true, 1, false, true);
}
template <int FX>
__global__ void __launch_bounds__(WG)
  k_syrk5_finish(const uint32_t *part, int nsplit, size_t part_stride, const uint32_t *tile_list, size_t total, const uint32_t *toomU,
                 uint32_t *acc, size_t acc_stride, int N, int col0, int col1)
{
  constexpr int A3 = fx_part_limbs<FX>(), Z = T5_Z, W = 2 * FX + 2, WB = toom_wb<FX>(), H = T5_H;
  const size_t pidx = (size_t)blockIdx.x * WG + threadIdx.x;
  int i, j;
  if(pidx >= total || !syrk_packed_decode<syrk_tile_edge<FX>()>(pidx, tile_list, N, col0, col1, i, j))
    return;
  const size_t idx = (size_t)i + (size_t)j * N;
  uint32_t V[9][Z];
#pragma unroll
  for(int q = 0; q < 9; ++q)
    {
      uint32_t g3[3][A3 + 1];
#pragma unroll
      for(int u = 0; u < 3; ++u)
        {
          uint64_t cy = 0;
#pragma unroll
          for(int k = 0; k < A3; ++k)
            {
              for(int sp = 0; sp < nsplit; ++sp)
                cy += part[(((size_t)sp * 27 + 3 * q + u) * A3 + k) * part_stride + pidx];
              g3[u][k] = (uint32_t)cy;
              cy >>= 32;
            }
          g3[u][A3] = (uint32_t)cy;
        }
      sub_limbs<A3 + 1>(g3[2], g3[0]);
      sub_limbs<A3 + 1>(g3[2], g3[1]);
#pragma unroll
      for(int k = 0; k < Z; ++k)
        V[q][k] = k < A3 + 1 ? g3[0][k < A3 + 1 ? k : 0] : 0u;
      add_shifted<Z, A3 + 1>(V[q], g3[2], H, false);
      add_shifted<Z, A3 + 1>(V[q], g3[1], 2 * H, false);
    }
  {
    uint32_t u[Z];
#pragma unroll
    for(int t = 0; t < 3; ++t)
      {
        const int q = 2 + 2 * t;
#pragma unroll
        for(int k = 0; k < Z; ++k)
          u[k] = toomU[(size_t)(t * Z + k) * N + i];
        z_sub<Z>(V[q], u);
#pragma unroll
        for(int k = 0; k < Z; ++k)
          u[k] = toomU[(size_t)(t * Z + k) * N + j];
        z_sub<Z>(V[q], u);
      }
  }
  constexpr int MI[7][9] = {{-700, -700, 350, 35, -7, 14, -10, -2, 6300},      {-1890, -80, -80, 1, 1, 4, 4, 0, -360},
                            {3150, 2750, -1175, -155, 29, -23, 5, 9, -28350},  {378, 68, 68, -1, -1, -1, -1, 0, 378},
                            {-3150, -1450, -125, 145, -19, 13, 5, -9, 28350},  {-360, -80, -80, 4, 4, 1, 1, 0, -1890},
                            {2100, 700, 350, -70, -14, -7, -5, 6, -18900}};
  constexpr int SH[7] = {2, 3, 3, 3, 3, 3, 2};
  constexpr uint32_t ODD[7] = {525, 45, 225, 9, 225, 45, 1575};
  uint32_t gg[W];
#pragma unroll
  for(int k = 0; k < W; ++k)
    gg[k] = k < Z ? V[0][k < Z ? k : 0] : 0u;
#pragma unroll
  for(int r = 0; r < 7; ++r)
    {
      uint32_t c[Z];
#pragma unroll
      for(int k = 0; k < Z; ++k)
        c[k] = 0;
#pragma unroll
      for(int q = 0; q < 9; ++q)
        if(MI[r][q] != 0)
          z_addmul<Z>(c, V[q], (uint32_t)(MI[r][q] < 0 ? -MI[r][q] : MI[r][q]), MI[r][q] < 0);
      z_sar<Z>(c, SH[r]);
      z_divexact<Z>(c, ODD[r], inv_mod_2_32(ODD[r]));
      add_shifted<W, Z>(gg, c, (r + 1) * WB, false);
    }
  add_shifted<W, Z>(gg, V[8], 8 * WB, false);
#pragma unroll
  for(int k = 0; k < W; ++k)
    acc[(size_t)k * acc_stride + idx] = gg[k];
}

template <int FX> constexpr int syrk_waves_per_simd() { return fx_toom4k<FX>() ? SDPB_SYRK3_WAVES : SDPB_SYRK_WAVES; }

template <int W> __global__ void __launch_bounds__(WG) k_acc_add_tri(uint32_t *dst, const uint32_t *src, size_t stride, int N)
{
  const size_t idx = (size_t)blockIdx.x * WG + threadIdx.x;
  if(idx >= (size_t)N * N + N)
    return;
  if(idx < (size_t)N * N && idx % N < idx / N)
    return;
  uint64_t cy = 0;
#pragma unroll
  for(int k = 0; k < W; ++k)
    {
      const uint64_t t = (uint64_t)dst[(size_t)k * stride + idx] + src[(size_t)k * stride + idx] + cy;
      dst[(size_t)k * stride + idx] = (uint32_t)t;
      cy = t >> 32;
    }
}

template <int FX>
__global__ void __launch_bounds__(WG) k_syrk_unbias(uint32_t *acc, size_t acc_stride, int N, unsigned long long nrows_total, size_t idx0, size_t idx1)
{
  constexpr int W = 2 * FX + 2, FB = fx_frac_bits<FX>();
  const size_t idx = idx0 + (size_t)blockIdx.x * WG + threadIdx.x;
  if(idx >= idx1)
    return;
  const int i = (int)(idx % N), j = (int)(idx / N);
  if(i < j)
    return;
  uint32_t w[W], s[W];
#pragma unroll
  for(int k = 0; k < W; ++k)
    w[k] = acc[(size_t)k * acc_stride + idx];
// ... 751 lines not shown
```

sdpb_amd/csrc/solver.hpp:

```cpp
#pragma once
#include "kernels.hpp"
#include "syrk_stage.hpp"
#include "mw_host.hpp"

#include <algorithm>
#include <atomic>
#include <chrono>
#include <cstring>
#include <limits>
#include <map>
#include <memory>
#include <sstream>
#include <string>
#include <utility>

namespace sdpb
{
struct SolverError : std::runtime_error
{
  int code;
  SolverError(int c, const std::string &m) : std::runtime_error(m), code(c) {}
};

struct Collectives
// ... 484 lines not shown
      << ", \"tiles_per_chunk\": " << pl.chunk_tiles << ", \"row_splits\": " << pl.nsplit_first
      << ", \"rows_per_split\": " << (pl.nsplit_first ? cdiv(qwin.chunk_rows, pl.nsplit_first) : 0) << ", \"planes_per_split\": " << Syrk::SYRK_PART_PLANES
      << ", \"partial_bytes\": " << pl.part_words * sizeof(uint32_t) << ", \"partial_bytes_unbounded\": " << unbounded.part_words * sizeof(uint32_t)
      << ", \"partial_bytes_full_square_layout\": "
      << (size_t)unbounded.nsplit_first * Syrk::SYRK_PART_PLANES * ((size_t)N_ * N_ + N_) * sizeof(uint32_t) * (unbounded.uses_part ? 1 : 0)
      << ", \"budget_bytes\": " << part_budget * sizeof(uint32_t) << ", \"budget_source\": \"" << syrk_.budget_source(false)
      << "\", \"bound_exceeded_min_chunk\": " << (pl.uses_part && pl.part_words > part_budget ? "true" : "false")
      << ", \"min_chunk_bytes\": " << Syrk::TILE_WORDS * sizeof(uint32_t) << "}"
      << ", \"image\": {\"image_chunks\": " << qwin.chunks << ", \"rows_per_chunk\": " << qwin.chunk_rows << ", \"rows\": " << Ptot_
      << ", \"image_bytes\": " << qwin.image_words * sizeof(uint32_t) << ", \"image_bytes_unbounded\": " << Syrk::image_words_for(std::max<size_t>(Ptot_, 1), (size_t)N_) * sizeof(uint32_t)
      << ", \"budget_bytes\": " << qwin.budget_words * sizeof(uint32_t) << ", \"budget_source\": \"" << syrk_.budget_source(true)
      << "\", \"bound_exceeded_min_chunk\": " << (qwin.bound_exceeded ? "true" : "false") << ", \"accumulator_bytes\": " << syrk_.acc2.n * sizeof(uint32_t)
      << ", \"last_call_windows\": " << rec.last_windows << "}"
      << ", \"window_budget_bytes\": " << syrk_.window_budget_words() * sizeof(uint32_t)
      << ", \"last_syrk_call\": {\"tiles\": " << rec.last_plan.ntile << ", \"chunks\": " << rec.last_plan.nchunk
      << ", \"tiles_per_chunk\": " << rec.last_plan.chunk_tiles << ", \"row_splits\": " << rec.last_plan.nsplit_first
      << ", \"partial_bytes\": " << rec.last_plan.part_words * sizeof(uint32_t) << "}"
      << ", \"device\": {\"free_bytes\": " << free_b << ", \"total_bytes\": " << total_b << "}}";
    return o.str();
  }
  void request_stop() override { stop_requested_.store(1); }
  long host_syncs() const override { return host_syncs_; }
  void progress(unsigned long long out[8]) const override
  {
    out[0] = prog_iteration_.load();
    out[1] = prog_syncs_.load();
    out[2] = seq_count_.load(std::memory_order_acquire);
    out[3] = seq_hash_.load();
    out[4] = seq_last_kind_.load();
    out[5] = seq_last_bytes_.load();
    out[6] = seq_last_root_.load();
    out[7] = comm_ ? (unsigned long long)comm_->async_error() : 0ull;
  }
  int terminate_reason() const override { return terminate_reason_; }

private:
  void build_layout()
  {
    size_t off_scaled = 0, off_psd = 0, off_bases = 0, off_E = 0, off_pair = 0, off_schur = 0, off_bt = 0, off_vecn = 0;
    for(int j = 0; j < J_; ++j)
      {
        const int m = dims_[j], K = npts_[j];
        const int n0 = m * ((K + 1) / 2), n1 = m * K - n0;
        total_psd_rows_ += n0 + n1;
        Ptot_global_ += (unsigned long long)K * m * (m + 1) / 2;
        if(owner_[j] != rank_)
          continue;
        local_.push_back(j);
        BlockDesc bd;
        bd.m = m;
        bd.K = K;
        bd.P = K * m * (m + 1) / 2;
        const int d = K - 1;
        bd.rows[0] = d / 2 + 1;
        bd.rows[1] = (d + 1) / 2;
        bd.n[0] = n0;
        bd.n[1] = n1;
        bd.voff = Ptot_;
        bd.global_index = j;
        blk_.push_back(bd);
        for(int b = 0; b < 2; ++b)
          {
            const int n = bd.n[b], q = m * K;
            h_psd_.push_back(MatDesc{off_psd, n, n, n, K});
            h_vecn_.push_back(MatDesc{off_vecn, n, 1, n, K});
            h_bases_.push_back(MatDesc{off_bases, bd.rows[b], K, bd.rows[b], K});
            h_basesT_.push_back(MatDesc{off_bases, K, bd.rows[b], K, K});
            const int pr = m * (m + 1) / 2;
            h_scaled_.push_back(MatDesc{off_scaled, K, pr * bd.rows[b], K, K});
            off_scaled += (size_t)K * pr * bd.rows[b];
            max_scaled_ = std::max(max_scaled_, (size_t)K * pr * bd.rows[b]);
            h_E_.push_back(MatDesc{off_E, n, q, n, K});
            h_Et_.push_back(MatDesc{off_E, q, n, q, K});
            h_pair_.push_back(MatDesc{off_pair, q, q, q, K});
            off_psd += (size_t)n * n;
            off_vecn += n;
            off_bases += (size_t)bd.rows[b] * K;
            off_E += (size_t)n * q;
            off_pair += (size_t)q * q;
            max_n_ = std::max(max_n_, n);
            max_q_ = std::max(max_q_, q);
          }
        h_schur_.push_back(MatDesc{off_schur, bd.P, bd.P, bd.P, K});
        h_bt_.push_back(MatDesc{off_bt, N_, bd.P, N_, K});
        h_vecP_.push_back(MatDesc{(unsigned long long)Ptot_, bd.P, 1, bd.P, K});
        off_schur += (size_t)bd.P * bd.P;
        off_bt += (size_t)N_ * bd.P;
        Ptot_ += bd.P;
        max_P_ = std::max(max_P_, bd.P);
        max_pairs_ = std::max(max_pairs_, m * (m + 1) / 2);
      }
    Jl_ = (int)local_.size();
    psd_elems_ = off_psd;
    psd_rows_local_ = off_vecn;

    d_blk_.upload(blk_);
    d_psd_.upload(h_psd_);
    d_vecn_.upload(h_vecn_);
    d_bases_.upload(h_bases_);
    d_basesT_.upload(h_basesT_);
    d_scaled_.upload(h_scaled_);
    d_E_.upload(h_E_);
    d_Et_.upload(h_Et_);
    d_pair_.upload(h_pair_);
    d_schur_.upload(h_schur_);
    d_bt_.upload(h_bt_);
    d_vecP_.upload(h_vecP_);
    d_Q_.upload(std::vector<MatDesc>{MatDesc{0, N_, N_, N_, 0}});
    d_vecQ_.upload(std::vector<MatDesc>{MatDesc{0, N_, 1, N_, 0}});

    q_nb_ = PB;
    q_panels_ = (N_ + q_nb_ - 1) / q_nb_;
    std::vector<MatDesc> qd;
    for(int p = 0; p < q_panels_; ++p)
      {
        const int k0 = p * q_nb_, nb = std::min(q_nb_, N_ - k0);
        qd.push_back(MatDesc{(unsigned long long)k0 + (unsigned long long)k0 * N_, nb, nb, N_, 0});
      }
    d_qdiag_.upload(qd);
    {
      std::vector<MatDesc> rows;
      for(const MatDesc &v : h_vecP_)
        rows.push_back(MatDesc{v.off, 1, v.rows, 1, v.aux});
      d_rowP_.upload(rows);
    }

    for(DevArray *a : {&X_, &Y_, &Xc_, &Yc_, &dX_, &dY_, &PR_, &mXY_, &R_, &Z_, &W_, &LiX_, &LiY_})
      a->alloc(off_psd, NL);
    bases_.alloc(off_bases, NL);
    basesT_.alloc(off_bases, NL);
    scaled_.alloc(off_scaled, NL);
    for(DevArray *a : {&E_, &Et_, &T_, &YQ_})
      a->alloc(off_E, NL);
    AX_.alloc(off_pair, NL);
    AY_.alloc(off_pair, NL);
    S_.alloc(off_schur, NL);
    LiS_.alloc(off_schur, NL);
    BT_.alloc(off_bt, NL);
    PT_.alloc(off_bt, NL);
    for(DevArray *a : {&c_, &x_, &dx_, &dres_, &invdS_})
      a->alloc(Ptot_, NL);
    for(DevArray *a : {&invdX_, &invdY_, &eigD_, &eigE_, &eigD2_, &eigE2_})
      a->alloc(off_vecn, NL);
    for(DevArray *a : {&b_, &y_, &dy_, &rp_, &norms_, &invnorms_, &invdQ_})
      a->alloc(N_, NL);
    Q_.alloc((size_t)N_ * N_, NL);
    eigF_.alloc(2 * (off_vecn + 1));
    eigF2_.alloc(2 * (off_vecn + 1));
    LiQ_.alloc((size_t)N_ * N_, NL);
    qtmpv_.alloc(N_, NL);
    part_.alloc((size_t)std::max(Jl_, 1) * N_, NL);
    red_.alloc(1024, NL);
    red2_.alloc(4, NL);
    lam_.alloc(std::max(2 * Jl_, 1), NL);
    lam2_.alloc(std::max(2 * Jl_, 1), NL);
    ratio_.alloc((size_t)5 * std::max(Jl_, 1) + 1, NL);
    scal_.alloc(S_COUNT, NL);
    if constexpr(td_trsm_enabled<NL>())
      {
        use_td_ = true;
        if(const char *e = std::getenv("SDPB_HIP_TILEDOT"))
          use_td_ = std::atoi(e) != 0;
        std::vector<int> off;
        size_t tiles = 0;
        for(const BlockDesc &bd : blk_)
          {
            off.push_back((int)tiles);
            const int nt = td_tiles_of(bd.P);
            tiles += nt;
            td_max_tiles_ = std::max(td_max_tiles_, nt);
          }
        use_td_ = use_td_ && tiles > 0;
        if(use_td_)
          {
            constexpr size_t WT = td::limbs<NL>();
            td_tile_off_.upload(off);
            td_img_.alloc(tiles * PB * PB * WT);
            td_sum_.alloc(tiles * PB * WT);
            td_exp_.alloc(tiles * PB);
          }
      }
    if(world_ > 1)
      acc64_.alloc(((size_t)N_ * (N_ + 1) / 2 + N_) * Syrk::ACCW);
    flags_.alloc((size_t)2 * std::max(Jl_, 1) + 4);
    flags2_.alloc((size_t)2 * std::max(Jl_, 1));
    flags3_.alloc((size_t)std::max(Jl_, 1));
    resbuf_.alloc(RES_WORDS);
    if(world_ > 1)
      xgather_.alloc(std::max(RES_WORDS, (size_t)(NL + 1) * N_) * world_);
    if(const char *e = std::getenv("SDPB_HIP_PROFILE"))
      profile_ = std::atoi(e) != 0;
    if(const char *e = std::getenv("SDPB_HIP_OVERLAP_SYRK"))
      overlap_syrk_ = std::atoi(e) != 0;
    if(const char *e = std::getenv("SDPB_HIP_TEST_SEQ_FAULT"))
      seq_fault_rank_ = std::atoi(e);
    if(const char *e = std::getenv("SDPB_HIP_QSOLVE_SUM_LANES"))
      qsolve_sum_lanes_ = std::atoi(e) != 0;
    if(const char *e = std::getenv("SDPB_HIP_TRIDIAG_WIDE"))
      tridiag_wide_ = std::atoi(e) != 0;
    {
      std::vector<int> ids;
      for(int pass = 0; pass < 2; ++pass)
        for(int q = 0; q < 2 * Jl_; ++q)
          if((h_psd_[q].rows > TRI_SMALL_N) == (pass == 0))
            ids.push_back(q);
      tri_count_large_ = 0;
      for(int q = 0; q < 2 * Jl_; ++q)
        tri_count_large_ += h_psd_[q].rows > TRI_SMALL_N;
      tri_ids_.upload(ids);
      if(const char *e = std::getenv("SDPB_HIP_TRI_T_SMALL"))
        tri_lanes_small_ = std::max(64, std::atoi(e));
      if(const char *e = std::getenv("SDPB_HIP_TRI_T_LARGE"))
        tri_lanes_large_ = std::max(64, std::atoi(e));
    }
    dist_cholq_ = false;
    if(const char *e = std::getenv("SDPB_HIP_DIST_CHOLQ"))
      dist_cholq_ = world_ > 1 && std::atoi(e) != 0;
    if(dist_cholq_)
      qpanel_msg_.alloc(((size_t)N_ * PB + (size_t)PB * PB + PB) * (NL + 1) + 2);
    part2_.alloc((size_t)std::max(Jl_, 1) * N_, NL);
    {
      const int panels = (int)cdiv(N_, PB), step = PB % 16 == 0 ? 1 : (PB % 8 == 0 ? 2 : (PB % 4 == 0 ? 4 : (PB % 2 == 0 ? 8 : 16)));
      bool want = false;
      if(const char *e = std::getenv("SDPB_HIP_Q_CHASE"))
        want = std::atoi(e) != 0;
      chase_hA_ = std::max(step, (panels / 2) / step * step);
      chase_cA_ = PB * chase_hA_;
      q_chase_ = want && !dist_cholq_ && !(overlap_syrk_ && world_ == 1) && chase_hA_ < panels && chase_cA_ < N_;
    }
    prepare_syrk();
  }
  void prepare_syrk() { syrk_.prepare(Ptot_, N_, stream_, q_chase_, q_chase_ ? chase_cA_ : 0); }

  void set_default_params()
  {
    set_param("dualityGapThreshold", "1e-30");
    set_param("primalErrorThreshold", "1e-30");
    set_param("dualErrorThreshold", "1e-30");
    set_param("initialMatrixScalePrimal", "1e20");
    set_param("initialMatrixScaleDual", "1e20");
    set_param("feasibleCenteringParameter", "0.1");
    set_param("infeasibleCenteringParameter", "0.3");
    set_param("stepLengthReduction", "0.7");
    set_param("maxComplementarity", "1e100");
    set_param("minPrimalStep", "0");
    set_param("minDualStep", "0");
  }

  Batch psd(const DevArray &a) const { return Batch{a.ptr(), d_psd_.p, 2 * Jl_}; }
  Batch vecn(const DevArray &a) const { return Batch{a.ptr(), d_vecn_.p, 2 * Jl_}; }
  Batch basesB() const { return Batch{bases_.ptr(), d_bases_.p, 2 * Jl_}; }
  Batch basesTB() const { return Batch{basesT_.ptr(), d_basesT_.p, 2 * Jl_}; }
  Batch scaledB() const { return Batch{scaled_.ptr(), d_scaled_.p, 2 * Jl_}; }
  Batch eB(const DevArray &a) const { return Batch{a.ptr(), d_E_.p, 2 * Jl_}; }
  Batch etB(const DevArray &a) const { return Batch{a.ptr(), d_Et_.p, 2 * Jl_}; }
  Batch pairB(const DevArray &a) const { return Batch{a.ptr(), d_pair_.p, 2 * Jl_}; }
  Batch schurB() const { return Batch{S_.ptr(), d_schur_.p, Jl_}; }
  Batch btB(const DevArray &a) const { return Batch{a.ptr(), d_bt_.p, Jl_}; }
  Batch vecPB(const DevArray &a) const { return Batch{a.ptr(), d_vecP_.p, Jl_}; }
  Batch QB() const { return Batch{Q_.ptr(), d_Q_.p, 1}; }
  Batch vecQB(const DevArray &a) const { return Batch{a.ptr(), d_vecQ_.p, 1}; }

  struct Timer
  {
    Solver *s;
    std::string name;
    std::chrono::steady_clock::time_point t0;
    Timer(Solver *s_, const char *n) : s(s_)
    {
      if(!s->profile_)
        return;
      name = n;
      t0 = std::chrono::steady_clock::now();
    }
    ~Timer()
    {
      if(!s->profile_ || name.empty())
        return;
      (void)hipStreamSynchronize(s->stream_);
      const double ms = std::chrono::duration<double, std::milli>(std::chrono::steady_clock::now() - t0).count();
      if(!s->timers_ms_.count(name))
        s->timer_order_.emplace_back(name, 0.0);
      s->timers_ms_[name] += ms;
    }
  };

public:
  std::string timers_json() override
  {
    HIP_CHECK(hipStreamSynchronize(stream_));
    resolve_syrk_events();
    std::ostringstream ss;
    ss << "{";
    bool first = true;
    for(auto &kv : timer_order_)
      {
        ss << (first ? "" : ", ") << "\"" << kv.first << "\": " << timers_ms_.at(kv.first);
        first = false;
      }
    const double fx_bytes = (double)Ptot_ * N_ * (FX + 1) * 4.0, acc_bytes = (double)N_ * (N_ + 1) / 2 * Syrk::ACCW * 4.0;
    ss << (first ? "" : ", ") << "\"kernel.k_syrk_fx.ms\": " << syrk_kernel_ms_ << ", \"kernel.k_syrk_fx.launches\": " << syrk_launches_
       << ", \"kernel.k_syrk_fx.algorithmic_bytes\": " << (fx_bytes + acc_bytes)
       << ", \"kernel.k_syrk_fx.limb_macs\": "
       << (double)Ptot_ * N_ * (N_ + 1) / 2 * FX * FX * (Syrk::SYRK_TOOM5K ? 27.0 / 64 : Syrk::SYRK_TOOM4K ? 21.0 / 64 : Syrk::SYRK_TOOM4 ? 7.0 / 16 : Syrk::SYRK_TWO_LEVEL ? 9.0 / 16 : 0.75)
       << ", \"kernel.k_syrk_fx.karatsuba_levels\": " << (Syrk::SYRK_TOOM4 ? 0 : Syrk::SYRK_TWO_LEVEL ? 2 : 1) << ", \"kernel.k_syrk_fx.toom4\": " << (Syrk::SYRK_TOOM4 ? 1 : 0) << ", \"kernel.k_syrk_fx.toom4k\": " << (Syrk::SYRK_TOOM4K ? 1 : 0) << ", \"kernel.k_syrk_fx.toom5k_lazy_carries\": " << (Syrk::SYRK_TOOM5K ? 1 : 0)
       << ", \"host_syncs\": " << host_syncs_ << ", \"launches\": " << launches_
       << ", \"iterations\": " << iteration_ << ", \"comm.world\": " << world_ << ", \"comm.ranks\": " << (comm_ ? comm_->ranks() : (world_ == 1 ? 1 : 0))
       << ", \"comm.owned_blocks\": " << Jl_ << ", \"comm.owned_rows\": " << Ptot_ << ", \"comm.allgather_calls\": " << xc_allgather_calls_
       << ", \"comm.allgather_bytes\": " << xc_allgather_bytes_ << ", \"comm.allreduce_calls\": " << xc_allreduce_calls_
       << ", \"comm.allreduce_bytes\": " << xc_allreduce_bytes_ << ", \"comm.broadcast_calls\": " << xc_broadcast_calls_
       << ", \"comm.broadcast_bytes\": " << xc_broadcast_bytes_ << ", \"comm.cholesky_Q\": " << (dist_cholq_ ? "\"distributed\"" : "\"replicated\"") << ", \"comm.q_chase\": " << (q_chase_ ? 1 : 0)
       << ", \"comm.collectives\": " << seq_count_.load() << ", \"comm.sequence_hash\": \"" << std::hex << seq_hash_.load() << std::dec << "\"";
    ss << "}";
    return ss.str();
  }

  void set_param(const std::string &n, const char *value) override
  {
    const M v = mw::from_decimal<NL>(value);
    if(n == "dualityGapThreshold") duality_gap_threshold_ = v;
    else if(n == "primalErrorThreshold") primal_error_threshold_ = v;
    else if(n == "dualErrorThreshold") dual_error_threshold_ = v;
    else if(n == "initialMatrixScalePrimal") initial_matrix_scale_primal_ = v;
    else if(n == "initialMatrixScaleDual") initial_matrix_scale_dual_ = v;
    else if(n == "feasibleCenteringParameter") feasible_centering_parameter_ = v;
    else if(n == "infeasibleCenteringParameter") infeasible_centering_parameter_ = v;
    else if(n == "stepLengthReduction") step_length_reduction_ = v;
    else if(n == "maxComplementarity") max_complementarity_ = v;
    else if(n == "minPrimalStep") min_primal_step_ = v;
    else if(n == "minDualStep") min_dual_step_ = v;
    else throw SolverError(4, "unknown parameter " + n);
  }
  void set_flags(long max_iterations, bool fpf, bool fdf, bool dpfj, bool ddfj) override
  {
    max_iterations_ = max_iterations;
    find_primal_feasible_ = fpf;
    find_dual_feasible_ = fdf;
    detect_primal_feasible_jump_ = dpfj;
    detect_dual_feasible_jump_ = ddfj;
  }

  std::vector<M> parse_list(const char *txt, size_t expect, const char *what)
  {
    std::vector<std::pair<const char *, const char *>> tok;
    split_numbers(txt, tok);
    if(tok.size() != expect)
      throw SolverError(4, std::string("wrong element count for ") + what + ": got " + std::to_string(tok.size())
                             + ", expected " + std::to_string(expect));
    std::vector<M> v(expect);
    for(size_t i = 0; i < expect; ++i)
      v[i] = mw::from_decimal<NL>(tok[i].first, tok[i].second);
    return v;
  }
  int local_index(int j) const
  {
    for(int l = 0; l < Jl_; ++l)
      if(local_[l] == j)
        return l;
    return -1;
  }

  void set_block(int j, const char *be, const char *bo, const char *B, const char *c) override
  {
    const int l = set_block_bases(j, be, bo);
    if(l < 0)
      return;
    const BlockDesc &bd = blk_[l];
    upload<NL>(BT_, h_bt_[l].off, parse_list(B, (size_t)bd.P * N_, "B"));
    upload<NL>(c_, bd.voff, parse_list(c, bd.P, "c"));
  }
  void set_block_f64(int j, const char *be, const char *bo, const double *B, const double *c) override
  {
    const int l = set_block_bases(j, be, bo);
    if(l < 0)
      return;
    const BlockDesc &bd = blk_[l];
    std::vector<M> v((size_t)bd.P * N_);
    for(size_t i = 0; i < v.size(); ++i)
      v[i] = mw::from_double<NL>(B[i]);
    upload<NL>(BT_, h_bt_[l].off, v);
    v.resize(bd.P);
    for(int i = 0; i < bd.P; ++i)
      v[i] = mw::from_double<NL>(c[i]);
    upload<NL>(c_, bd.voff, v);
  }
  static std::vector<M> records(const uint64_t *rec, size_t count, int limbs64)
  {
    if(!rec || limbs64 < 1)
      throw SolverError(4, "mpf records: null pointer or limbs64 < 1");
    std::vector<M> v(count);
    try
      {
        for(size_t i = 0; i < count; ++i)
          v[i] = mw::from_mpf_record<NL>(rec + i * (size_t)(limbs64 + 2), limbs64);
      }
    catch(std::exception &e)
      {
        throw SolverError(4, e.what());
      }
    return v;
  }
  void set_block_mpf(int j, int limbs64, const uint64_t *be, const uint64_t *bo, const uint64_t *B, const uint64_t *c) override
  {
    if(j < 0 || j >= J_)
      throw SolverError(4, "set_block: block index out of range");
    const int l = local_index(j);
    if(l < 0)
      return;
    const BlockDesc &bd = blk_[l];
    const std::vector<M> e = records(be, (size_t)bd.rows[0] * bd.K, limbs64), o = records(bo, (size_t)bd.rows[1] * bd.K, limbs64);
    set_block_bases_values(l, e, o);
    upload<NL>(BT_, h_bt_[l].off, records(B, (size_t)bd.P * N_, limbs64));
    upload<NL>(c_, bd.voff, records(c, bd.P, limbs64));
  }
  void set_objective_mpf(int limbs64, const uint64_t *b, const uint64_t *constant) override
  {
    upload<NL>(b_, 0, records(b, N_, limbs64));
    objective_const_ = records(constant, 1, limbs64)[0];
  }
  int set_block_bases(int j, const char *be, const char *bo)
  {
    if(j < 0 || j >= J_)
      throw SolverError(4, "set_block: block index out of range");
    const int l = local_index(j);
    if(l < 0)
      return -1;
    const BlockDesc &bd = blk_[l];
    set_block_bases_values(l, parse_list(be, (size_t)bd.rows[0] * bd.K, "bilinear_bases"), parse_list(bo, (size_t)bd.rows[1] * bd.K, "bilinear_bases"));
    return l;
  }
  void set_block_bases_values(int l, const std::vector<M> &even, const std::vector<M> &odd)
  {
    const BlockDesc &bd = blk_[l];
    const std::vector<M> *src[2] = {&even, &odd};
    for(int b = 0; b < 2; ++b)
      {
        const int rs = bd.rows[b];
        const std::vector<M> &v = *src[b];
        std::vector<M> cm((size_t)rs * bd.K);
        for(int r = 0; r < rs; ++r)
          for(int k = 0; k < bd.K; ++k)
            cm[(size_t)k * rs + r] = v[(size_t)r * bd.K + k];
        upload<NL>(bases_, h_bases_[2 * l + b].off, cm);
        upload<NL>(basesT_, h_basesT_[2 * l + b].off, v);
      }
    Batch bb = basesB(), ee = eB(E_), et = etB(Et_);
    bb.d += 2 * l;
    ee.d += 2 * l;
    et.d += 2 * l;
    bb.count = ee.count = et.count = 2;
    const size_t mx = std::max((size_t)bd.n[0] * bd.m * bd.K, (size_t)bd.n[1] * bd.m * bd.K);
    launch(k_build_bases_block<NL>, dim3(cdiv(mx, WG), 2), dim3(WG), stream_, bb, ee, et, d_blk_.p + l);
    HIP_CHECK(hipStreamSynchronize(stream_));
  }
  void set_objective(const char *b, const char *constant) override
  {
    upload<NL>(b_, 0, parse_list(b, N_, "b"));
    objective_const_ = mw::from_decimal<NL>(constant);
  }

  void init_state() override
  {
    LaunchScope launches_of_this_solver(&launches_);
    for(DevArray *a : {&X_, &Y_, &x_, &y_, &dx_, &dy_, &dX_, &dY_})
      HIP_CHECK(hipMemsetAsync(a->base, 0, a->bytes(), stream_));
    upload_scalar(S_ALPHA_P, initial_matrix_scale_primal_);
    upload_scalar(S_ALPHA_D, initial_matrix_scale_dual_);
    add_diagonal(X_, S_ALPHA_P);
    add_diagonal(Y_, S_ALPHA_D);
    iteration_ = 0;
    started_ = false;
    terminate_reason_ = NotTerminated;
    primal_step_length_ = mw::zero<NL>();
    dual_step_length_ = mw::zero<NL>();
    HIP_CHECK(hipStreamSynchronize(stream_));
  }

private:
  mw::Ptr res() const { return mw::Ptr{resbuf_.p, (size_t)R_COUNT}; }
  uint32_t *xwords() const { return resbuf_.p + (size_t)(NL + 1) * R_COUNT; }
  void store_scalar(mw::Ptr p, size_t idx, const M &v) { launch(k_store_scalar<NL>, dim3(1), dim3(64), stream_, p, idx, v); }
  void upload_scalar(int slot, const M &v) { store_scalar(scal_.ptr(), (size_t)slot, v); }

  template <class F> void foreach(size_t count, F f)
  {
    if(!count)
      return;
    launch(k_foreach<F>, dim3(std::min<unsigned>(cdiv(count, WG), 4096)), dim3(WG), stream_, count, f);
  }
  template <int OP, class F> void reduce_to(int slot, size_t count, F f, const M &empty = mw::zero<NL>())
  {
    if(!count)
      {
        store_scalar(res(), (size_t)slot, empty);
        return;
      }
    const unsigned g = std::min<unsigned>(cdiv(count, WG), 512);
    launch(k_reduce<NL, OP, F>, dim3(g), dim3(WG), stream_, count, f, red_.ptr());
    mw::CPtr rp = red_.cptr();
    auto ld = [rp] __device__(size_t i) { return mw::load<NL>(rp, i); };
    launch(k_reduce<NL, OP, decltype(ld)>, dim3(1), dim3(WG), stream_, (size_t)g, ld, mw::Ptr{resbuf_.p + slot, (size_t)R_COUNT});
  }
  Comm &comm()
  {
    if(!comm_)
      throw SolverError(4, "world_size > 1 but no collectives were registered (sdpb_hip_set_collectives / sdpb_hip_rccl_init)");
    return *comm_;
  }
  void exchange(std::initializer_list<std::pair<int, int>> slot_ops)
  {
    if(world_ == 1)
      return;
    XOps ops;
    for(int &o : ops.op)
      o = X_KEEP;
    for(auto &so : slot_ops)
      ops.op[so.first] = so.second;
    xc_allgather_calls_ += 1;
    xc_allgather_bytes_ += (double)(RES_WORDS * sizeof(uint32_t));
    note_collective(COLL_ALLGATHER, RES_WORDS * sizeof(uint32_t), -1);
    {
      unsigned long long h = seq_hash_.load();
      if(seq_fault_rank_ == rank_)
        h ^= 1ull;
      launch(k_store_words2<0>, dim3(1), dim3(64), stream_, xwords() + XW_SEQ_LO, (uint32_t)h, (uint32_t)(h >> 32));
    }
    comm().allgather(resbuf_.p, xgather_.p, RES_WORDS * sizeof(uint32_t), stream_);
    launch(k_combine_slots<NL>, dim3(1), dim3(64), stream_, (const uint32_t *)xgather_.p, world_, (int)R_COUNT, ops, resbuf_.p);
  }
  void fetch(unsigned max_stage = FAIL_Q)
  {
    uint32_t h[RES_WORDS];
    HIP_CHECK(hipMemcpyAsync(h, resbuf_.p, sizeof h, hipMemcpyDeviceToHost, stream_));
    HIP_CHECK(hipStreamSynchronize(stream_));
    host_syncs_ += 1;
    prog_syncs_.store((unsigned long long)host_syncs_);
    for(int i = 0; i < R_COUNT; ++i)
      {
        const uint32_t hd = h[i];
        res_host_[i].neg = hd >> 31;
        res_host_[i].e = hd ? (int32_t)((hd & 0x7fffffffu) - mw::EBIAS) : mw::EZERO;
        for(int k = 0; k < NL; ++k)
          res_host_[i].m[k] = h[(size_t)(k + 1) * R_COUNT + i];
      }
    for(int k = 0; k < X_EXTRA; ++k)
      xw_host_[k] = h[(size_t)(NL + 1) * R_COUNT + k];
    throw_if_failed(max_stage);
  }
  void throw_if_failed(unsigned max_stage)
  {
    if(world_ > 1 && xw_host_[XW_SEQBAD])
      {
        (void)hipStreamSynchronize(stream_q_);
        (void)hipStreamSynchronize(stream_q2_);
        q_pending_ = false;
        std::ostringstream ss;
        ss << "collective sequence mismatch: rank " << (xw_host_[XW_SEQBAD] - 1) << " and rank 0 enqueued different (kind, bytes, root) "
           << "sequences on the exchange before synchronisation point " << host_syncs_ << " of iteration " << iteration_
           << " (this rank: " << seq_count_.load() << " collectives)";
        throw HipError(3, ss.str());
      }
    const uint32_t tag = xw_host_[XW_FAIL];
    if(tag == 0xffffffffu || (tag >> 27) > max_stage)
      return;
    (void)hipStreamSynchronize(stream_q_);
    (void)hipStreamSynchronize(stream_q2_);
    q_pending_ = false;
    const unsigned stage = tag >> 27, code = tag & ((1u << 27) - 1u);
    std::ostringstream ss;
    switch(stage)
      {
      case FAIL_X:
      case FAIL_Y:
        ss << "Error when computing Cholesky decomposition of Block_Diagonal_Matrix " << (stage == FAIL_X ? "X" : "Y")
           << ", block index = " << code / 2 << ", parity = " << code % 2 << ": A was not numerically HPD";
        break;
      case FAIL_S:
        ss << "Error when computing Cholesky decomposition of block_" << code << ": A was not numerically HPD";
        break;
      case FAIL_QDIAG:
        ss << "Normalized Q should have ones on diagonal. For i = " << code;
        break;
      default:
        ss << "Error when computing Cholesky(Q): A was not numerically HPD";
      }
    throw SolverError(1, ss.str());
  }
  void allreduce_vec_sum(DevArray &a, size_t count)
  {
    if(world_ == 1)
      return;
    if(a.n != count)
      throw SolverError(4, "allreduce_vec_sum: array stride differs from the vector length");
    const size_t words = (size_t)(NL + 1) * count;
    if(xgather_.n < words * world_)
      {
        HIP_CHECK(hipDeviceSynchronize());
        xgather_.alloc(words * world_);
      }
    xc_allgather_calls_ += 1;
    xc_allgather_bytes_ += (double)(words * sizeof(uint32_t));
    note_collective(COLL_ALLGATHER, words * sizeof(uint32_t), -1);
    comm().allgather(a.base, xgather_.p, words * sizeof(uint32_t), stream_);
    launch(k_combine_vec<NL>, dim3(cdiv(count, WG)), dim3(WG), stream_, (const uint32_t *)xgather_.p, world_, (int)count, a.ptr());
  }
  struct OnSideStream
  {
// ... 1360 lines not shown
```

sdpb_amd/csrc/syrk_stage.hpp:

```cpp
#pragma once
#include "kernels.hpp"

namespace sdpb
{
inline std::vector<uint32_t> syrk_tile_order(int N, int split_col = 0, int *count_left = nullptr, int edge = 16)
{
  int SB = edge == 16 ? 8 : 4;
  if(const char *env = std::getenv("SDPB_HIP_SYRK_SB"))
    SB = std::max(1, std::atoi(env));
  const int tiles = (N + edge - 1) / edge, nsb = (tiles + SB - 1) / SB;
  std::vector<uint32_t> all;
  for(int bi = 0; bi < nsb; ++bi)
    for(int bj = 0; bj <= bi; ++bj)
      for(int ti = bi * SB; ti < std::min(tiles, (bi + 1) * SB); ++ti)
        for(int tj = bj * SB; tj < std::min(tiles, (bj + 1) * SB); ++tj)
          if(tj <= ti)
            all.push_back((uint32_t)ti << 16 | (uint32_t)tj);
  if(split_col <= 0)
    {
      if(count_left)
        *count_left = (int)all.size();
      return all;
    }
  std::vector<uint32_t> out;
  for(uint32_t t : all)
    if((int)(t & 0xffffu) * edge < split_col)
      out.push_back(t);
  if(count_left)
    *count_left = (int)out.size();
  for(uint32_t t : all)
    if(((int)(t & 0xffffu) + 1) * edge > split_col)
      out.push_back(t);
  return out;
}

constexpr int SYRK_MAX_SPLITS = 32;
inline int syrk_row_splits(int ntile, unsigned nrows, int slots, int rb, unsigned max_rows = 0)
{
  if(const char *env = std::getenv("SDPB_HIP_SYRK_SPLITS"))
    return std::max(1, std::min(SYRK_MAX_SPLITS, std::atoi(env)));
  int smin = 1;
  while(max_rows && smin < SYRK_MAX_SPLITS && nrows / (unsigned)smin > max_rows && nrows / (unsigned)(smin + 1) >= 64u * (unsigned)rb)
    ++smin;
  int best = smin;
  double best_eff = 0;
  for(int s = smin; s <= SYRK_MAX_SPLITS; ++s)
    {
      if(s > smin && nrows / (unsigned)s < 64u * (unsigned)rb)
        break;
      const double items = (double)ntile * s, rounds = std::ceil(items / slots), eff = items / (rounds * slots);
      if(eff > best_eff + 0.02)
        {
          best = s;
          best_eff = eff;
        }
    }
  return best;
}

struct SyrkPlan
{
  int ntile = 0, chunk_tiles = 0, nchunk = 0;
  int nsplit_first = 1;
  size_t part_words = 0;
  bool uses_part = false;
};
struct QWindow
{
  unsigned chunk_rows = 0;
  int chunks = 0;
  size_t stride = 0;
  size_t image_words = 0;
  size_t budget_words = 0;
  bool bound_exceeded = false;
};
struct SyrkRecord
{
  size_t default_words = 0;
  size_t max_shared_bytes = 0;
  SyrkPlan last_plan;
  int last_windows = 1;
};

template <int FX> class FxSyrk
{
public:
  static constexpr int ACCW = 2 * FX + 2;
  static constexpr bool SYRK_TOOM4 = fx_toom4<FX>();
  static constexpr bool SYRK_TOOM4K = fx_toom4k<FX>();
  static constexpr bool SYRK_TOOM5K = fx_toom5k<FX>();
  static constexpr int SYRK_NPROD = fx_nprod<FX>();
  static constexpr int SYRK_EDGE = syrk_tile_edge<FX>();
  static constexpr unsigned SYRK_SPLIT_ROWS = SYRK_TOOM4K ? 2560u : 0u;
  static constexpr bool SYRK_TWO_LEVEL = fx_two_level<FX>() || SYRK_TOOM4;
  static constexpr int SYRK_PART_PLANES = SYRK_TOOM4K ? SYRK_NPROD * fx_part_limbs<FX>() : SYRK_TOOM4 ? 7 * (2 * (FX / 4) + 1) : ACCW;
  static constexpr size_t TOOMU_WORDS = SYRK_TOOM5K ? (size_t)3 * T5_Z : (size_t)2 * (2 * (FX / 4) + 2);
  static constexpr size_t COLSUM_WORDS = SYRK_TOOM5K ? 25 : FX + 8;
#ifndef SDPB_SYRK2_RBG
#define SDPB_SYRK2_RBG (FX >= 32 ? 16 : 32)
#endif
  static constexpr int SYRK_RB = SYRK_TWO_LEVEL ? SDPB_SYRK2_RBG : (FX <= 24 ? 16 : 8);
  static constexpr size_t TILE_WORDS = (size_t)SYRK_PART_PLANES * SYRK_EDGE * SYRK_EDGE;

  explicit FxSyrk(int num_cus) : num_cus_(num_cus), rec_(&own_) {}
  explicit FxSyrk(const FxSyrk *solver_stage) : num_cus_(solver_stage->num_cus_), rec_(solver_stage->rec_) {}

  void set_max_shared_memory(size_t bytes) { rec_->max_shared_bytes = bytes; }
  size_t window_budget_words() const { return rec_->max_shared_bytes ? std::max<size_t>(1, rec_->max_shared_bytes / sizeof(uint32_t)) : rec_->default_words; }
  size_t syrk_part_budget_words(size_t image_words) const
  {
    if(const char *e = std::getenv("SDPB_HIP_SYRK_PART_BYTES"))
      return std::max<size_t>(1, (size_t)std::max(1.0, std::atof(e)) / sizeof(uint32_t));
    const size_t w = window_budget_words();
    return std::max<size_t>(1, w - std::min(image_words, w / 2));
  }
  size_t syrk_part_budget_words() const { return syrk_part_budget_words(win.image_words); }
  size_t image_budget_words() const
  {
    if(const char *e = std::getenv("SDPB_HIP_SYRK_IMAGE_BYTES"))
      return std::max<size_t>(1, (size_t)std::max(1.0, std::atof(e)) / sizeof(uint32_t));
    return std::max<size_t>(1, window_budget_words() / 2);
  }
  const char *budget_source(bool image) const
  {
    if(std::getenv(image ? "SDPB_HIP_SYRK_IMAGE_BYTES" : "SDPB_HIP_SYRK_PART_BYTES"))
      return image ? "SDPB_HIP_SYRK_IMAGE_BYTES" : "SDPB_HIP_SYRK_PART_BYTES";
    if(rec_->max_shared_bytes)
      return image ? "maxSharedMemory/2" : "maxSharedMemory";
    return image ? "device/2" : "device";
  }
  const SyrkRecord &record() const { return *rec_; }

  static size_t image_stride(size_t rows, size_t cols) { return std::max<size_t>(1, fx_image_stride<FX>(rows, cols, SYRK_RB)); }
  static size_t image_words_for(size_t rows, size_t cols) { return image_stride(rows, cols) * fx_planes<FX>() + 4; }
  static unsigned colsum_slices(size_t rows) { return (unsigned)std::min<size_t>(128, std::max<size_t>(1, cdiv(rows, 64))); }
  static int syrk_group_split()
  {
    if(!SYRK_TOOM4K)
      return 1;
    if(const char *e = std::getenv("SDPB_HIP_SYRK_GSPLIT"))
      {
        const int g = std::atoi(e);
        return g == 1 ? 1 : (g == 7 || g == 9) ? SYRK_NPROD / 3 : SYRK_NPROD;
      }
    return SYRK_NPROD;
  }
  int syrk_splits_for(int tiles, unsigned nrows, size_t budget_words) const
  {
    const int slots = num_cus_ * syrk_waves_per_simd<FX>();
    int nsplit = syrk_row_splits(tiles * syrk_group_split(), nrows, slots, SYRK_RB, SYRK_SPLIT_ROWS);
    const size_t per_split = TILE_WORDS * tiles;
    if(budget_words && (size_t)nsplit * per_split > budget_words)
      nsplit = (int)std::max<size_t>(1, budget_words / per_split);
    while(nsplit > 1 && (size_t)(nsplit - 1) * (cdiv(cdiv(nrows, nsplit), SYRK_RB) * SYRK_RB) >= nrows)
      --nsplit;
    return nsplit;
  }
  SyrkPlan syrk_plan(int ntile, unsigned nrows, size_t budget_words) const
  {
    SyrkPlan pl;
    pl.ntile = ntile;
    const int nsplit_all = syrk_splits_for(ntile, nrows, 0);
    pl.uses_part = nsplit_all > 1 || SYRK_TOOM4;
    pl.chunk_tiles = ntile;
    pl.nchunk = ntile ? 1 : 0;
    pl.nsplit_first = nsplit_all;
    if(!pl.uses_part || !ntile)
      return pl;
    const size_t need = (size_t)nsplit_all * TILE_WORDS * ntile;
    if(budget_words && need > budget_words)
      {
        const size_t bw = std::max(budget_words, TILE_WORDS);
        int nchunk = (int)cdiv(need, bw);
        for(;; ++nchunk)
          {
            int ct = (int)cdiv(ntile, nchunk);
            if(ct >= 64)
              ct = (int)(cdiv(ct, 8) * 8);
            pl.chunk_tiles = std::min(ntile, ct);
            pl.nsplit_first = syrk_splits_for(pl.chunk_tiles, nrows, bw);
            if((size_t)pl.nsplit_first * TILE_WORDS * pl.chunk_tiles <= bw || pl.chunk_tiles <= 1)
              break;
          }
        pl.nchunk = (int)cdiv(ntile, pl.chunk_tiles);
      }
    pl.part_words = (size_t)pl.nsplit_first * TILE_WORDS * pl.chunk_tiles;
    return pl;
  }
  QWindow q_window(unsigned nrows, int N, bool one_chunk = false) const
  {
    QWindow w;
    w.budget_words = image_budget_words();
    const unsigned quantum = (unsigned)SYRK_RB;
    unsigned rows = std::max(nrows, 1u);
    if(!one_chunk && image_words_for(rows, (size_t)N) > w.budget_words)
      {
        const size_t per_row = fx_row_slots<FX>((size_t)N) * fx_planes<FX>();
        const size_t fixed = (size_t)64 * fx_planes<FX>() + 4;
        size_t fit = w.budget_words > fixed ? (w.budget_words - fixed) / per_row : 0;
        fit = fit / quantum * quantum;
        if(fit < quantum)
          {
            fit = quantum;
            w.bound_exceeded = true;
          }
        const unsigned f = (unsigned)cdiv(nrows, fit);
        unsigned cr = (unsigned)(cdiv(cdiv(nrows, f), quantum) * quantum);
        if(SYRK_SPLIT_ROWS && cr > SYRK_SPLIT_ROWS)
          {
            const unsigned up = (unsigned)(cdiv(cr, SYRK_SPLIT_ROWS) * SYRK_SPLIT_ROWS);
            if(up <= fit)
              cr = up;
          }
        rows = cr;
      }
    if(one_chunk && image_words_for(rows, (size_t)N) > w.budget_words)
      w.bound_exceeded = true;
    w.chunk_rows = rows;
    w.chunks = nrows ? (int)cdiv(nrows, rows) : 1;
    w.stride = image_stride((size_t)rows, (size_t)N);
    w.image_words = w.stride * fx_planes<FX>() + 4;
    return w;
  }

  DevBuf<uint32_t> image, acc, acc2, colsum_partial, toomU, tiles, part, zero_piece;
  QWindow win;
  size_t acc_stride = 0;
  struct Tiles { int first, count, col0, col1; };
  Tiles all() const { return Tiles{0, ntile_, 0, cols_}; }
  Tiles left() const { return Tiles{0, ntile_left_, 0, split_col_}; }
  Tiles right() const { return Tiles{ntile_left_, ntile_ - ntile_left_, split_col_, cols_}; }
  int plan_tiles() const { return std::max(ntile_left_, ntile_ - ntile_left_); }

  void prepare(size_t rows, int cols, hipStream_t stream, bool one_chunk = false, int split_col = 0)
  {
    auto fit = [](DevBuf<uint32_t> &b, size_t words) {
      if(b.n != std::max<size_t>(words, 1))
        b.alloc(words);
    };
    if(cols != cols_ || split_col != split_col_ || !tiles.p)
      {
        const std::vector<uint32_t> order = syrk_tile_order(cols, split_col, &ntile_left_, SYRK_EDGE);
        ntile_ = (int)order.size();
        tiles.upload(order);
      }
    rows_ = rows, cols_ = cols, split_col_ = split_col;
    acc_stride = (size_t)cols * cols + cols;
    fit(acc, acc_stride * ACCW);
    if(SYRK_TOOM4)
      fit(toomU, TOOMU_WORDS * cols);
    fit(colsum_partial, (size_t)colsum_slices(rows) * COLSUM_WORDS * cols);
    fit(zero_piece, 64);
    if(!rec_->default_words)
      {
        size_t free_b = 0, total_b = 0;
        HIP_CHECK(hipMemGetInfo(&free_b, &total_b));
        const size_t reserve = total_b / 16 + ((size_t)1 << 30);
        const size_t b = std::min(free_b > reserve ? free_b - reserve : 0, total_b / 8);
        rec_->default_words = std::max<size_t>(b, (size_t)64 << 20) / sizeof(uint32_t);
      }
    win = q_window((unsigned)rows, cols, one_chunk);
    if(image.n != win.image_words)
      {
        image.alloc(win.image_words);
        HIP_CHECK(hipMemsetAsync(image.p, 0, image.n * sizeof(uint32_t), stream));
      }
    if(win.chunks > 1)
      fit(acc2, acc_stride * ACCW);
    const size_t budget = syrk_part_budget_words();
    const size_t words = std::max(syrk_plan(ntile_left_, win.chunk_rows, budget).part_words,
                                  syrk_plan(ntile_ - ntile_left_, win.chunk_rows, budget).part_words);
    if(words)
      fit(part, words);
  }

  void column_sums(hipStream_t stream) { column_sums(stream, acc.p, (unsigned)rows_); }
  void G(hipStream_t stream, const Tiles &t) { G(stream, t, acc.p, (unsigned)rows_); }
  template <class MakeImage, class Mark> void G_windows(hipStream_t stream, MakeImage &&make, Mark &&mark)
  {
    for(int c = 0; c < win.chunks; ++c)
      {
        const size_t r0 = (size_t)c * win.chunk_rows;
        const unsigned rows = (unsigned)std::min<size_t>(win.chunk_rows, rows_ - r0);
        if(c > 0 && rows < win.chunk_rows)
          HIP_CHECK(hipMemsetAsync(image.p, 0, image.n * sizeof(uint32_t), stream));
        make(r0, rows);
        uint32_t *out = c == 0 ? acc.p : acc2.p;
        column_sums(stream, out, rows);
        if(c == 0)
          mark();
        G(stream, all(), out, rows);
        if(c > 0)
          launch(k_acc_add_tri<ACCW>, dim3(cdiv(acc_stride, WG)), dim3(WG), stream, acc.p, (const uint32_t *)acc2.p, acc_stride, cols_);
      }
    rec_->last_windows = win.chunks;
  }

private:
  int num_cus_;
  SyrkRecord own_, *rec_;
  size_t rows_ = 0;
  int cols_ = 0, split_col_ = 0, ntile_ = 0, ntile_left_ = 0;

  void column_sums(hipStream_t stream, uint32_t *out, unsigned nrows)
  {
    const unsigned slices = colsum_slices(nrows), rows_per_slice = cdiv(nrows, slices);
    const uint32_t *fx = image.p;
    uint32_t *partial = colsum_partial.p;
    const int N = cols_;
    const dim3 grid(cdiv(N, 64), slices), final_grid(cdiv(N, WG));
    if constexpr(SYRK_TOOM4)
      {
        if constexpr(SYRK_TOOM5K)
          {
            launch(k_fx_colsum5<FX>, grid, dim3(WG), stream, fx, win.stride, nrows, N, rows_per_slice, partial);
            launch(k_fx_colsum5_final<FX>, final_grid, dim3(WG), stream, (const uint32_t *)partial, (int)slices, N, out, acc_stride, toomU.p,
                   (unsigned long long)nrows);
            return;
          }
        launch(k_fx_colsum2<FX, true>, grid, dim3(WG), stream, fx, win.stride, nrows, N, rows_per_slice, partial);
        launch(k_fx_colsum4_final<FX>, final_grid, dim3(WG), stream, (const uint32_t *)partial, (int)slices, N, out, acc_stride, toomU.p,
               (unsigned long long)nrows);
        return;
      }
    else if constexpr(SYRK_TWO_LEVEL)
      {
        launch(k_fx_colsum2<FX>, grid, dim3(WG), stream, fx, win.stride, nrows, N, rows_per_slice, partial);
        launch(k_fx_colsum2_final<FX>, final_grid, dim3(WG), stream, (const uint32_t *)partial, (int)slices, N, out, acc_stride);
        return;
      }
    launch(k_fx_colsum<FX>, grid, dim3(WG), stream, fx, win.stride, nrows, N, rows_per_slice, partial);
    launch(k_fx_colsum_final<FX>, final_grid, dim3(WG), stream, (const uint32_t *)partial, (int)slices, N, out, acc_stride);
  }
  void G(hipStream_t stream, const Tiles &t, uint32_t *out_acc, unsigned nrows)
  {
    const int ntile = t.count, N = cols_, col0 = t.col0, col1 = t.col1;
    if(ntile == 0 || col1 <= col0)
      return;
    const int gsplit = syrk_group_split();
    const SyrkPlan pl = syrk_plan(ntile, nrows, syrk_part_budget_words());
    if(pl.uses_part && part.n < pl.part_words)
      part.alloc(pl.part_words);
    rec_->last_plan = pl;
    const uint32_t *fx = image.p, *tu = toomU.p;
    constexpr size_t TW = (size_t)SYRK_EDGE * SYRK_EDGE;
    for(int t0 = 0; t0 < ntile; t0 += pl.chunk_tiles)
      {
        const int nt = std::min(pl.chunk_tiles, ntile - t0);
        const uint32_t *tl = tiles.p + t.first + t0;
        const int nsplit = nt == pl.chunk_tiles ? pl.nsplit_first : std::min(pl.nsplit_first, syrk_splits_for(nt, nrows, pl.part_words));
        const unsigned rps = cdiv(cdiv(nrows, nsplit), SYRK_RB) * SYRK_RB;
        const size_t ps = (size_t)nt * TW, total = ps;
        const bool packed = pl.uses_part;
        uint32_t *out = packed ? part.p : out_acc;
        const size_t os = packed ? ps : acc_stride;
        const dim3 grid(8 * cdiv((size_t)nt * nsplit, 8)), finish_grid(cdiv(total, WG));
        if constexpr(SYRK_TOOM4)
          {
            if constexpr(SYRK_TOOM4K)
              launch(k_syrk_fx3<FX, SYRK_RB>, dim3(8 * cdiv((size_t)nt * nsplit * gsplit, 8)), dim3(WG), stream, fx, win.stride, nrows, N, out, os, tl,
                     nt, nsplit, rps, gsplit);
            else
              launch(k_syrk_fx2<FX, SYRK_RB, true>, grid, dim3(WG), stream, fx, win.stride, nrows, N, out, os, tl, nt, nsplit, rps,
                     (const uint32_t *)zero_piece.p, 1);
            int nsum = nsplit;
            if constexpr(SYRK_TOOM4K)
              if(nsplit > 1)
                {
                  launch(k_syrk3_sum_splits<FX>, dim3(cdiv(total, WG), SYRK_NPROD), dim3(WG), stream, part.p, nsplit, ps, tl, total, N, col0, col1);
                  nsum = 1;
                }
            if constexpr(SYRK_TOOM5K)
              launch(k_syrk5_finish<FX>, finish_grid, dim3(WG), stream, (const uint32_t *)part.p, nsum, ps, tl, total, tu, out_acc, acc_stride, N,
                     col0, col1);
            else
              launch(k_syrk4_finish<FX>, finish_grid, dim3(WG), stream, (const uint32_t *)part.p, nsum, ps, tl, total, tu, out_acc, acc_stride, N,
                     col0, col1);
            continue;
          }
        else if constexpr(SYRK_TWO_LEVEL)
          launch(k_syrk_fx2<FX, SYRK_RB>, grid, dim3(WG), stream, fx, win.stride, nrows, N, out, os, tl, nt, nsplit, rps,
                 (const uint32_t *)zero_piece.p, (int)packed);
        else
          launch(k_syrk_fx<FX, SYRK_RB>, grid, dim3(WG), stream, fx, win.stride, nrows, N, out, os, tl, nt, nsplit, rps, (int)packed);
        if(packed)
          launch(k_syrk_reduce<FX>, finish_grid, dim3(WG), stream, (const uint32_t *)part.p, nsplit, ps, tl, total, out_acc, acc_stride, N, col0,
                 col1);
      }
  }
};
}
```

sdpb_amd/workmodel.py:

```python
from __future__ import annotations

from typing import Dict, Sequence


def shapes(dims: Sequence[int], num_points: Sequence[int]):
    for m, K in zip(dims, num_points):
        P = K * m * (m + 1) // 2
        n0 = m * ((K + 1) // 2)
        n1 = m * K - n0
        yield m, K, P, (n0, n1), m * K


def macs_per_iteration(dims, num_points, N) -> Dict[str, float]:
    w = dict(cholesky_XY=0.0, pairings=0.0, schur=0.0, schur_cholesky=0.0, schur_trsm=0.0, syrk_Q=0.0,
             cholesky_Q=0.0, XY=0.0, search_direction=0.0, step_length=0.0, residues=0.0)
    for m, K, P, ns, q in shapes(dims, num_points):
        for n in ns:
            w["cholesky_XY"] += 2 * n ** 3 / 3.0
            w["pairings"] += 2.5 * n * n * q + n * q * q
            w["XY"] += n ** 3
            w["search_direction"] += 2 * 7 * n ** 3
            w["step_length"] += 2 * (2 * n ** 3 + 6 * n ** 3)
            w["residues"] += n * n * K
        w["schur"] += 8.0 * P * P
        w["schur_cholesky"] += P ** 3 / 3.0
        w["schur_trsm"] += P * P * N / 2.0
        w["syrk_Q"] += P * N * (N + 1) / 2.0
        w["search_direction"] += 2 * (2 * P * P + 2 * P * N)
        w["residues"] += 2 * P * N
    w["cholesky_Q"] = N ** 3 / 3.0
    w["search_direction"] += 2 * 2 * N * N
    w["total"] = sum(w.values())
    return w


def algorithmic_bytes_per_iteration(dims, num_points, N, bytes_per_number: int) -> float:
    t = 0.0
    for m, K, P, ns, q in shapes(dims, num_points):
        for n in ns:
            t += 2 * n * n + 2 * q * q
        t += 4 * q * q + P * P
        t += P * P + 2 * P * N
        t += P * N
    t += N * (N + 1) / 2 + N * N
    return t * bytes_per_number


COMPILED_LIMBS = (6, 10, 16, 18, 24, 26, 34, 42, 50, 66)
HBM_BYTES = 288 * 10 ** 9


def limbs_for(precision: int) -> int:
    want = 2 * ((precision + 127) // 64)
    for nl in COMPILED_LIMBS:
        if nl >= want:
            return nl
    raise ValueError(f"--precision {precision} is beyond the compiled widths")


def _fx(nl: int):
    fx = nl - 2
    if fx >= 14 and fx % 4:
        fx += 4 - fx % 4
    toom4 = fx >= 16 and fx % 4 == 0
    toom4k = fx in (16, 24, 32)
    toom5k = fx == 16
    two = fx % 4 == 0
    words = 54 if toom5k else 21 * (fx // 8) if toom4k else 7 * (fx // 4) if toom4 else 9 * (fx // 4) if two else 3 * (fx // 2)
    planes = 135 if toom5k else 21 * (2 * (fx // 8) + 1) if toom4k else 7 * (2 * (fx // 4) + 1) if toom4 else 2 * fx + 2
    rb = (16 if fx >= 32 else 32) if two else (16 if fx <= 24 else 8)
    waves = 3 if toom4k else (3 if fx <= 16 else 2)
    return fx, words, 32 if toom4k else 16, planes, rb, waves, toom4, toom4k


def syrk_row_splits(ntile: int, nrows: int, slots: int, rb: int, max_rows: int) -> int:
    import math
    smin = 1
    while max_rows and smin < 32 and nrows // smin > max_rows and nrows // (smin + 1) >= 64 * rb:
        smin += 1
    best, best_eff = smin, 0.0
    for s in range(smin, 33):
        if s > smin and nrows // s < 64 * rb:
            break
        items = ntile * s
        eff = items / (math.ceil(items / slots) * slots)
        if eff > best_eff + 0.02:
            best, best_eff = s, eff
    return best


def q_window(rows: int, N: int, nl: int, image_budget_bytes: int):
    fx, words, edge, planes, rb, waves, toom4, toom4k = _fx(nl)

    slots = -(-N // 32) * 32 if fx == 16 else N

    def image_bytes(r):
        stride = (-(-r // rb) * rb * slots + 64) if toom4k else r * N
        return (max(stride, 1) * words + 4) * 4
    r = max(rows, 1)
    budget_words = max(1, image_budget_bytes // 4)
    if image_bytes(r) // 4 > budget_words:
        per_row = slots * words
        fixed = 64 * words + 4
        fit = ((budget_words - fixed) // per_row if budget_words > fixed else 0) // rb * rb
        fit = max(fit, rb)
        f = -(-rows // fit)
        cr = -(-(-(-rows // f)) // rb) * rb
        if toom4k and cr > 2560:
            up = -(-cr // 2560) * 2560
            if up <= fit:
                cr = up
        r = cr
    return r, (-(-rows // r) if rows else 1), image_bytes(r)


def planned_footprint(dims, num_points, N, precision, owners=None, rank=0, world=1, num_cus=256, hbm_bytes=HBM_BYTES,
                      max_shared_bytes=0, dist_cholq=False, free_bytes=None) -> Dict[str, float]:
    nl = limbs_for(precision)
    W = 4 * (nl + 1)
    fx, words, edge, planes, rb, waves, toom4, toom4k = _fx(nl)
    psd = bases = scaled = E = pair = schur = bt = vecn = rows = jl = 0
    for j, (m, K, P, ns, q) in enumerate(shapes(dims, num_points)):
        if owners is not None and owners[j] != rank:
            continue
        jl += 1
        d = K - 1
        pr = m * (m + 1) // 2
        for n, r in zip(ns, (d // 2 + 1, (d + 1) // 2)):
            psd += n * n
            vecn += n
            bases += r * K
            scaled += K * pr * r
            E += n * q
            pair += q * q
        schur += P * P
        bt += N * P
        rows += P
    out = {"psd_state_and_scratch": 13 * max(psd, 1) * W, "bases_and_pairings": (2 * max(bases, 1) + max(scaled, 1) + 4 * max(E, 1) + 2 * max(pair, 1)) * W,
           "schur_blocks": 2 * max(schur, 1) * W, "B": max(bt, 1) * W, "P": max(bt, 1) * W}
    accw = 2 * fx + 2
    q_bytes = 2 * N * N * W + (N * N + N) * accw * 4
    if world > 1:
        q_bytes += (N * (N + 1) // 2 + N) * accw * 8
        if dist_cholq:
            pb = 16 if nl > 34 else 32
            q_bytes += ((N * pb + pb * pb + pb) * (nl + 1) + 2) * 4
    out["Q"] = q_bytes
    out["vectors_and_small"] = (5 * max(rows, 1) + 6 * max(vecn, 1) + 8 * N + 2 * max(jl, 1) * N) * W
    rest = sum(out.values())
    free = (hbm_bytes if free_bytes is None else free_bytes) - rest
    reserve = hbm_bytes // 16 + (1 << 30)
    window = max_shared_bytes or max(min(max(free - reserve, 0), hbm_bytes // 8), 64 << 20)
    chunk_rows, windows, image = q_window(rows, N, nl, max(window // 2, 4))
    out["P_fixed_point_image"] = image
    if windows > 1:
        out["Q"] += (N * N + N) * accw * 4
    tiles = -(-N // edge)
    ntile = tiles * (tiles + 1) // 2

    def planes_unbounded(r):
        ns = syrk_row_splits(ntile * (21 if toom4k else 1), r, num_cus * waves, rb, 2560 if toom4k else 0) if r else 1
        return ns * planes * ntile * edge * edge * 4 if (ns > 1 or toom4) else 0
    unbounded = planes_unbounded(chunk_rows)
    budget = max(window - min(image, window // 2), 4)
    out["syrk_partial_planes"] = min(unbounded, max(budget, planes * edge * edge * 4))
    out["total"] = float(sum(out.values()))
    out["rows"] = rows
    out["owned_blocks"] = jl
    out["syrk_partial_planes_unbounded"] = planes_unbounded(rows)
    out["image_chunks"] = windows
    out["image_rows_per_chunk"] = chunk_rows
    out["window_budget_bytes"] = window
    return out
```

Measured before the change: 6.341.

## Split Toom-5 pieces with a second Karatsuba level and add dedicated syrk kernel

The Toom-5 fixed-point image now stores each 2-limb piece together with the sum of its limbs, giving 81 planes instead of 54. A new k_syrk5_k2 kernel launches 64-thread workgroups and performs an extra Karatsuba level per piece, so three 32-bit products replace four in each 2x2 limb product. It uses lazy 64-bit column accumulators with periodic carries, and each of the three sub-products is accumulated into the output plane in turn. The old lazy path in k_syrk_fx3 is removed. The change cuts multiply count by a quarter but costs a larger image (more memory traffic and footprint), extra read-modify-write passes over the accumulators, and a new occupancy and split model.

```diff
diff --git a/sdpb_amd/csrc/kernels.hpp b/sdpb_amd/csrc/kernels.hpp
--- a/sdpb_amd/csrc/kernels.hpp
+++ b/sdpb_amd/csrc/kernels.hpp
@@ -1706,13 +1706,13 @@
 template <int FX> constexpr int toom_wb() { return fx_toom5k<FX>() ? 102 : 32 * (FX / 4) - (fx_toom4k<FX>() ? 6 : 4); }
 template <int FX> constexpr int fx_planes()
 {
-  return fx_toom5k<FX>() ? 27 * 2 : fx_toom4k<FX>() ? 21 * (FX / 8) : fx_toom4<FX>() ? 7 * (FX / 4) : fx_two_level<FX>() ? 9 * (FX / 4) : 3 * (FX / 2);
+  return fx_toom5k<FX>() ? 27 * 3 : fx_toom4k<FX>() ? 21 * (FX / 8) : fx_toom4<FX>() ? 7 * (FX / 4) : fx_two_level<FX>() ? 9 * (FX / 4) : 3 * (FX / 2);
 }
 template <int FX> constexpr int fx_frac_bits()
 {
   return fx_toom5k<FX>() ? 5 * toom_wb<FX>() - 1 : fx_toom4<FX>() ? 4 * toom_wb<FX>() - 1 : fx_two_level<FX>() ? 32 * FX - 7 : 32 * FX - 3;
 }
-template <int FX> constexpr int fx_col_slot(int c) { return fx_toom5k<FX>() ? 32 * (c / 32) + 2 * (c % 16) + (c % 32) / 16 : c; }
+template <int FX> constexpr int fx_col_slot(int c) { return fx_toom5k<FX>() ? 32 * (c / 32) + 4 * (c % 8) + (c % 32) / 8 : c; }
 template <int FX> constexpr size_t fx_row_slots(size_t cols) { return fx_toom5k<FX>() ? (cols + 31) / 32 * 32 : cols; }
 template <int FX> MW_HD size_t fx_elem(size_t idx, int N)
 {
@@ -1985,6 +1985,7 @@
   constexpr int TOPBIT = WB - 32 * (ML - 1);
   static_assert(FB == 5 * WB - 1 && FB / 32 == FX - 1, "a' = v + 2^FB fills five pieces of WB bits");
   static_assert(TOPBIT >= 0 && TOPBIT + 7 <= 32 && WB + 7 <= 2 * H && H + 1 <= 2 * LB, "121 b fits, the halves fit two limbs");
+  static_assert(H - LB + 1 <= LB, "the upper limb of a half has H - LB bits, that of mid one more: every limb < 2^LB, their sum xm <= 2^(LB+1) - 2");
   uint32_t a[FX];
   uint64_t borrow = 0;
 #pragma unroll
@@ -2051,9 +2052,14 @@
       const uint32_t s0 = lo[0] + hi[0];
       mid[0] = s0 & T5_MASK;
       mid[1] = lo[1] + hi[1] + (s0 >> LB);
-      piece_store<2>(fx + ((size_t)(3 * g + 0) * fx_stride + idx) * 2, lo);
-      piece_store<2>(fx + ((size_t)(3 * g + 1) * fx_stride + idx) * 2, hi);
-      piece_store<2>(fx + ((size_t)(3 * g + 2) * fx_stride + idx) * 2, mid);
+      const uint32_t *piece[3] = {lo, hi, mid};
+#pragma unroll
+      for(int u = 0; u < 3; ++u)
+        {
+          fx[(size_t)(9 * g + 3 * u + 0) * fx_stride + idx] = piece[u][0];
+          fx[(size_t)(9 * g + 3 * u + 1) * fx_stride + idx] = piece[u][1];
+          fx[(size_t)(9 * g + 3 * u + 2) * fx_stride + idx] = piece[u][0] + piece[u][1];
+        }
     }
 }
 
@@ -3208,17 +3214,13 @@
 #ifndef SDPB_SYRK3_WAVES
 #define SDPB_SYRK3_WAVES 3
 #endif
-#ifndef SDPB_SYRK3_LAZY_TRIP
-#define SDPB_SYRK3_LAZY_TRIP 32
-#endif
 template <int FX, int RBG>
 __global__ void __launch_bounds__(WG, SDPB_SYRK3_WAVES)
   k_syrk_fx3(const uint32_t *__restrict__ fx_in, size_t fx_stride, unsigned nrows, int N, uint32_t *acc, size_t acc_stride,
              const uint32_t *tile_list, int ntile, int nsplit, unsigned rows_per_split, int gsplit)
 {
-  constexpr bool LAZY = fx_toom5k<FX>();
   constexpr int M3 = FX / 8, A3 = fx_part_limbs<FX>(), NPROD = fx_nprod<FX>();
-  static_assert(M3 >= 2 && M3 <= 4 && (!LAZY || (M3 == 2 && RBG <= 32)), "accumulators of 2 x 2 outputs in registers; 2 x 32 rows between carries");
+  static_assert(M3 >= 2 && M3 <= 4 && !fx_toom5k<FX>(), "accumulators of 2 x 2 outputs in registers");
   constexpr int ROWW = 32 * M3, UPR = ROWW / 4, NPAIR = RBG * UPR, GL = NPAIR / WG;
   static_assert(NPAIR % WG == 0, "a pass stages a whole number of units per lane");
   const uint32_t *fx = (const uint32_t *)__builtin_assume_aligned(fx_in, 4);
@@ -3241,7 +3243,6 @@
   __shared__ __attribute__((aligned(16))) uint32_t sb[2 * NPAIR * 4 + 64];
   uint64_t cc[4][2 * M3 - 1];
   uint32_t hh[4][2 * M3 - 1];
-  uint64_t dd[4][2 * M3 - 1];
 #if defined(__HIP_DEVICE_COMPILE__)
   constexpr bool DIRECT = true;
 #else
@@ -3307,12 +3308,10 @@
       {
 #if defined(__HIP_DEVICE_COMPILE__)
     typedef uint32_t u32x4 __attribute__((ext_vector_type(4)));
-    constexpr int LSTEP = LAZY ? 2 * M3 : M3;
-    const uint32_t la = (uint32_t)(uintptr_t)(__attribute__((address_space(3))) uint32_t *)(sa + buf * NPAIR * 4 + li * LSTEP);
-    const uint32_t lb = (uint32_t)(uintptr_t)(__attribute__((address_space(3))) uint32_t *)(sb + buf * NPAIR * 4 + lj * LSTEP);
+    const uint32_t la = (uint32_t)(uintptr_t)(__attribute__((address_space(3))) uint32_t *)(sa + buf * NPAIR * 4 + li * M3);
+    const uint32_t lb = (uint32_t)(uintptr_t)(__attribute__((address_space(3))) uint32_t *)(sb + buf * NPAIR * 4 + lj * M3);
     static_assert(RBG % 4 == 0 && M3 == 2, "four rows per trip, offsets in units of 8 bytes");
 #define FX3_P(C, H, X, Y) "v_mad_u64_u32 %" #C ", vcc, %" #X ", %" #Y ", %" #C "\n\tv_addc_co_u32 %" #H ", vcc, 0, %" #H ", vcc\n\t"
-#define FX3_L(C, X, Y) "v_mad_u64_u32 %" #C ", vcc, %" #X ", %" #Y ", %" #C "\n\t"
 #define FX3_MAC_BOTH(o0, o1, a0x, a0y, a1x, a1y, bx, by)                                                                                   \
   asm volatile(FX3_P(0, 6, 12, 16) FX3_P(3, 9, 14, 16) FX3_P(1, 7, 12, 17) FX3_P(4, 10, 14, 17) FX3_P(1, 7, 13, 16) FX3_P(4, 10, 15, 16)   \
                  FX3_P(2, 8, 13, 17) FX3_P(5, 11, 15, 17)                                                                                  \
@@ -3323,17 +3322,6 @@
 #define FX3_MAC_ONE(o0, ax, ay, bx, by)                                                                                                    \
   asm volatile(FX3_P(0, 3, 6, 8) FX3_P(1, 4, 6, 9) FX3_P(1, 4, 7, 8) FX3_P(2, 5, 7, 9)                                                     \
                : "+v"(c[o0][0]), "+v"(c[o0][1]), "+v"(c[o0][2]), "+v"(h[o0][0]), "+v"(h[o0][1]), "+v"(h[o0][2])                            \
-               : "v"(ax), "v"(ay), "v"(bx), "v"(by)                                                                                        \
-               : "vcc")
-#define FX3L_MAC_BOTH(o0, o1, a0x, a0y, a1x, a1y, bx, by)                                                                                  \
-  asm volatile(FX3_L(0, 6, 10) FX3_L(3, 8, 10) FX3_L(1, 6, 11) FX3_L(4, 8, 11) FX3_L(1, 7, 10) FX3_L(4, 9, 10) FX3_L(2, 7, 11)             \
-                 FX3_L(5, 9, 11)                                                                                                           \
-               : "+v"(c[o0][0]), "+v"(c[o0][1]), "+v"(c[o0][2]), "+v"(c[o1][0]), "+v"(c[o1][1]), "+v"(c[o1][2])                            \
-               : "v"(a0x), "v"(a0y), "v"(a1x), "v"(a1y), "v"(bx), "v"(by)                                                                  \
-               : "vcc")
-#define FX3L_MAC_ONE(o0, ax, ay, bx, by)                                                                                                   \
-  asm volatile(FX3_L(0, 3, 5) FX3_L(1, 3, 6) FX3_L(1, 4, 5) FX3_L(2, 4, 6)                                                                 \
-               : "+v"(c[o0][0]), "+v"(c[o0][1]), "+v"(c[o0][2])                                                                            \
                : "v"(ax), "v"(ay), "v"(bx), "v"(by)                                                                                        \
                : "vcc")
 #define FX3_QUADRANTS(BOTH, ONE, va, vb)                                                                                                   \
@@ -3355,89 +3343,43 @@
   else                                                                                                                                     \
     ONE(0, va.x, va.y, vb.x, vb.y);
 #define FX3_MACS(va, vb) FX3_QUADRANTS(FX3_MAC_BOTH, FX3_MAC_ONE, va, vb)
-#define FX3L_MACS(va, vb) FX3_QUADRANTS(FX3L_MAC_BOTH, FX3L_MAC_ONE, va, vb)
 #define FX3_NEXT(wa, wb, ra, rb, O0, O1)                                                                                                   \
   asm volatile("s_waitcnt lgkmcnt(0)\n\tds_read2_b64 %2, %4 offset0:" #O0 " offset1:" #O1 "\n\tds_read2_b64 %3, %5 offset0:" #O0            \
                " offset1:" #O1                                                                                                             \
                : "+v"(wa), "+v"(wb), "=&v"(ra), "=&v"(rb)                                                                                  \
                : "v"(xa), "v"(xb)                                                                                                          \
                : "memory")
-#define FX3L_NEXT(wa, wb, ra, rb, ROW)                                                                                                     \
-  asm volatile("s_waitcnt lgkmcnt(0)\n\tds_read_b128 %2, %4 offset:%6\n\tds_read_b128 %3, %5 offset:%6"                                   \
-               : "+v"(wa), "+v"(wb), "=&v"(ra), "=&v"(rb)                                                                                  \
-               : "v"(xa), "v"(xb), "n"((ROW) * 256)                                                                                        \
-               : "memory")
-#define FX3L_ROWS2(R)                                                                                                                      \
-  FX3L_NEXT(a0, b0, a1, b1, (R) + 1);                                                                                                      \
-  FX3L_MACS(a0, b0)                                                                                                                        \
-  FX3L_NEXT(a1, b1, a0, b0, (R) + 2);                                                                                                      \
-  FX3L_MACS(a1, b1)
-#define FX3L_ROWS8(R) FX3L_ROWS2(R) FX3L_ROWS2((R) + 2) FX3L_ROWS2((R) + 4) FX3L_ROWS2((R) + 6)
     u32x4 a0, b0, a1, b1;
-    if constexpr(LAZY)
+    {
+      const uint32_t xa = la, xb = lb;
+      asm volatile("ds_read2_b64 %0, %2 offset0:0 offset1:16\n\tds_read2_b64 %1, %3 offset0:0 offset1:16" : "=&v"(a0), "=&v"(b0) : "v"(xa), "v"(xb) : "memory");
+    }
+#pragma unroll 1
+    for(int rr = 0; rr < RBG; rr += 4)
       {
-        constexpr int TRIP = (RBG % SDPB_SYRK3_LAZY_TRIP == 0) ? SDPB_SYRK3_LAZY_TRIP : 8;
-        static_assert(RBG % 8 == 0 && (TRIP == 8 || TRIP == 16 || TRIP == 32) && RBG * 256 < 65536, "whole trips, the offsets fit 16 bits");
-        {
-          const uint32_t xa = la, xb = lb;
-          asm volatile("ds_read_b128 %0, %2\n\tds_read_b128 %1, %3" : "=&v"(a0), "=&v"(b0) : "v"(xa), "v"(xb) : "memory");
-        }
-#pragma unroll 1
-        for(int rr = 0; rr < RBG; rr += TRIP)
-          {
-            const uint32_t xa = la + rr * 256, xb = lb + rr * 256;
-            FX3L_ROWS8(0)
-            if constexpr(TRIP >= 16)
-              {
-                FX3L_ROWS8(8)
-              }
-            if constexpr(TRIP >= 32)
-              {
-                FX3L_ROWS8(16)
-                FX3L_ROWS8(24)
-              }
-          }
-      }
-    else
-      {
-        {
-          const uint32_t xa = la, xb = lb;
-          asm volatile("ds_read2_b64 %0, %2 offset0:0 offset1:16\n\tds_read2_b64 %1, %3 offset0:0 offset1:16" : "=&v"(a0), "=&v"(b0) : "v"(xa), "v"(xb) : "memory");
-        }
-#pragma unroll 1
-        for(int rr = 0; rr < RBG; rr += 4)
-          {
-            const uint32_t xa = la + rr * 256, xb = lb + rr * 256;
-            FX3_NEXT(a0, b0, a1, b1, 32, 48);
-            FX3_MACS(a0, b0)
-            FX3_NEXT(a1, b1, a0, b0, 64, 80);
-            FX3_MACS(a1, b1)
-            FX3_NEXT(a0, b0, a1, b1, 96, 112);
-            FX3_MACS(a0, b0)
-            FX3_NEXT(a1, b1, a0, b0, 128, 144);
-            FX3_MACS(a1, b1)
-          }
+        const uint32_t xa = la + rr * 256, xb = lb + rr * 256;
+        FX3_NEXT(a0, b0, a1, b1, 32, 48);
+        FX3_MACS(a0, b0)
+        FX3_NEXT(a1, b1, a0, b0, 64, 80);
+        FX3_MACS(a1, b1)
+        FX3_NEXT(a0, b0, a1, b1, 96, 112);
+        FX3_MACS(a0, b0)
+        FX3_NEXT(a1, b1, a0, b0, 128, 144);
+        FX3_MACS(a1, b1)
       }
     asm volatile("s_waitcnt lgkmcnt(0)" : "+v"(a0), "+v"(b0)::"memory");
-#undef FX3L_ROWS8
-#undef FX3L_ROWS2
-#undef FX3L_NEXT
 #undef FX3_NEXT
-#undef FX3L_MACS
 #undef FX3_MACS
 #undef FX3_QUADRANTS
-#undef FX3L_MAC_ONE
-#undef FX3L_MAC_BOTH
 #undef FX3_MAC_ONE
 #undef FX3_MAC_BOTH
 #undef FX3_P
-#undef FX3_L
 #endif
       }
     else
       {
-        constexpr int LSTEP = LAZY ? 2 * M3 : M3, SECOND = LAZY ? M3 : 16 * M3;
-        const uint32_t *pa = sa + buf * NPAIR * 4 + li * LSTEP, *pb = sb + buf * NPAIR * 4 + lj * LSTEP;
+        constexpr int SECOND = 16 * M3;
+        const uint32_t *pa = sa + buf * NPAIR * 4 + li * M3, *pb = sb + buf * NPAIR * 4 + lj * M3;
 #pragma unroll SDPB_SYRK2_UNROLL
         for(int rr = 0; rr < RBG; ++rr)
           {
@@ -3448,23 +3390,6 @@
               piece_load<M3>(pa + rr * ROWW + SECOND, a1);
             if constexpr((MASK & 12) != 0)
               piece_load<M3>(pb + rr * ROWW + SECOND, b1);
-            if constexpr(LAZY)
-              {
-                auto lazy = [&](const uint32_t (&x)[M3], const uint32_t (&y)[M3], uint64_t (&cs)[2 * M3 - 1]) {
-                  cs[0] += (uint64_t)x[0] * y[0];
-                  cs[1] += (uint64_t)x[0] * y[1] + (uint64_t)x[1] * y[0];
-                  cs[2] += (uint64_t)x[1] * y[1];
-                };
-                lazy(a0, b0, c[0]);
-                if constexpr((MASK & 2) != 0)
-                  lazy(a1, b0, c[1]);
-                if constexpr((MASK & 4) != 0)
-                  lazy(a0, b1, c[2]);
-                if constexpr((MASK & 8) != 0)
-                  lazy(a1, b1, c[3]);
-              }
-            else
-              {
             SyrkColumns<M3, 0>::run(a0, b0, c[0], h[0]);
             if constexpr((MASK & 2) != 0)
               SyrkColumns<M3, 0>::run(a1, b0, c[1], h[1]);
@@ -3472,7 +3397,6 @@
               SyrkColumns<M3, 0>::run(a0, b1, c[2], h[2]);
             if constexpr((MASK & 8) != 0)
               SyrkColumns<M3, 0>::run(a1, b1, c[3], h[3]);
-              }
           }
       }
   };
@@ -3486,33 +3410,6 @@
             cc[o][k] = 0;
             hh[o][k] = 0;
           }
-#pragma unroll
-      for(int o = 0; o < 4; ++o)
-#pragma unroll
-        for(int k = 0; k < 2 * M3 - 1; ++k)
-          dd[o][k] = 0;
-      auto carry_columns = [&](bool all) __attribute__((always_inline)) {
-        if constexpr(LAZY)
-          {
-#pragma unroll
-            for(int o = 0; o < 4; ++o)
-              {
-                dd[o][1] += cc[o][1] >> 32;
-                cc[o][1] &= 0xffffffffull;
-              }
-            if(all)
-              {
-#pragma unroll
-                for(int o = 0; o < 4; ++o)
-                  {
-                    dd[o][0] += cc[o][0] >> 32;
-                    cc[o][0] &= 0xffffffffull;
-                    dd[o][2] += cc[o][2] >> 32;
-                    cc[o][2] &= 0xffffffffull;
-                  }
-              }
-          }
-      };
       if(prod > prod_begin)
         __syncthreads();
       fetch(prod, row_begin, 0);
@@ -3520,14 +3417,10 @@
       __syncthreads();
       auto sweep = [&](auto mask_c) __attribute__((always_inline)) {
         int buf = 0;
-        unsigned pass = 0;
         for(unsigned r0 = row_begin; r0 < row_end; r0 += RBG)
           {
             fetch(prod, r0 + RBG < row_end ? r0 + RBG : row_begin, buf ^ 1);
             rows(mask_c, buf, cc, hh);
-            ++pass;
-            if(LAZY && (pass & 1u) == 0)
-              carry_columns((pass & 3u) == 0);
             store(buf ^ 1);
             __syncthreads();
             buf ^= 1;
@@ -3550,18 +3443,6 @@
 #pragma unroll
           for(int k = 0; k < A3; ++k)
             g[k] = 0;
-          if constexpr(LAZY)
-            {
-              unsigned __int128 v = 0;
-#pragma unroll
-              for(int k = 0; k < 2 * M3 - 1; ++k)
-                v += ((unsigned __int128)cc[o][k] + ((unsigned __int128)dd[o][k] << 32)) << (T5_LB * k);
-              g[0] = (uint32_t)v;
-              g[1] = (uint32_t)(v >> 32);
-              g[2] = (uint32_t)(v >> 64);
-              g[3] = (uint32_t)(v >> 96);
-            }
-          else
           syrk_fold<M3, A3>(g, cc[o], hh[o]);
           const size_t at = (size_t)tile * 1024 + (size_t)(li + 16 * (o & 1)) + (size_t)(lj + 16 * (o >> 1)) * 32;
 #pragma unroll
@@ -3569,6 +3450,280 @@
             acc[(size_t)(prod * A3 + k) * acc_stride + at] = g[k];
         }
     }
+}
+
+#ifndef SDPB_SYRK5_ROWS
+#define SDPB_SYRK5_ROWS 16
+#endif
+constexpr int SYRK5_WG = 64;
+constexpr uint32_t T5_XM_MAX = 2 * T5_MASK;
+constexpr unsigned SYRK5_CARRY_ROWS_XM = 64, SYRK5_CARRY_ROWS_X = 128;
+static_assert(((unsigned __int128)1 << 32) + (unsigned __int128)SYRK5_CARRY_ROWS_XM * T5_XM_MAX * T5_XM_MAX < ((unsigned __int128)1 << 64),
+              "a column of xm products: what a carry leaves (< 2^32) plus 64 rows stays below 2^64");
+static_assert(((unsigned __int128)1 << 32) + (unsigned __int128)SYRK5_CARRY_ROWS_X * T5_MASK * T5_MASK < ((unsigned __int128)1 << 64),
+              "a column of x0 or x1 products: what a carry leaves plus 128 rows stays below 2^64");
+constexpr int syrk5_wg_per_cu(int rows_per_pass) { return 160 * 1024 / (4 * 128 * rows_per_pass) < 16 ? 160 * 1024 / (4 * 128 * rows_per_pass) : 16; }
+template <int PN, bool DIAG> MW_HD void syrk5k2_mac_row(uint64_t (&c)[4][4], const uint32_t (&a)[4], const uint32_t (&b)[4])
+{
+#pragma unroll
+  for(int p = 0; p < PN; ++p)
+#pragma unroll
+    for(int q = 0; q < 4; ++q)
+      if(!DIAG || q <= p)
+        c[p][q] += (uint64_t)a[p] * b[q];
+}
+MW_HD void syrk5k2_carry(uint64_t (&c)[4][4], uint64_t (&d)[4][4])
+{
+#pragma unroll
+  for(int p = 0; p < 4; ++p)
+#pragma unroll
+    for(int q = 0; q < 4; ++q)
+      {
+        d[p][q] += c[p][q] >> 32;
+        c[p][q] &= 0xffffffffull;
+      }
+}
+template <int RBG> MW_HD void syrk5k2_pass_end(int t, unsigned &since, uint64_t (&c)[4][4], uint64_t (&d)[4][4])
+{
+  static_assert(SYRK5_CARRY_ROWS_XM % RBG == 0 && SYRK5_CARRY_ROWS_X % RBG == 0, "the carry cadences are whole passes");
+  since += RBG;
+  if(since >= (t == 2 ? SYRK5_CARRY_ROWS_XM : SYRK5_CARRY_ROWS_X))
+    {
+      syrk5k2_carry(c, d);
+      since = 0;
+    }
+}
+MW_HD unsigned __int128 syrk5k2_term(int t, uint64_t c, uint64_t d)
+{
+  const unsigned __int128 s = (unsigned __int128)c + ((unsigned __int128)d << 32);
+  return t == 0 ? s - (s << T5_LB) : t == 1 ? (s << (2 * T5_LB)) - (s << T5_LB) : s << T5_LB;
+}
+
+template <int FX, int RBG>
+__global__ void __launch_bounds__(SYRK5_WG)
+  k_syrk5_k2(const uint32_t *__restrict__ fx_in, size_t fx_stride, unsigned nrows, int N, uint32_t *acc, size_t acc_stride,
+             const uint32_t *tile_list, int ntile, int nsplit, unsigned rows_per_split, int gsplit)
+{
+  constexpr int A3 = fx_part_limbs<FX>(), NPROD = fx_nprod<FX>();
+  static_assert(fx_toom5k<FX>() && A3 == 5 && (RBG == 16 || RBG == 32), "one-word planes of the lazy-carry image; whole 16-byte units per lane and pass");
+  constexpr int UNITS = RBG * 8, GL = UNITS / SYRK5_WG;
+  const uint32_t *fx = (const uint32_t *)__builtin_assume_aligned(fx_in, 4);
+  const int nitem = ntile * nsplit * gsplit, per = (nitem + 7) / 8;
+  const int item = (int)(blockIdx.x % 8) * per + (int)(blockIdx.x / 8);
+  if((int)(blockIdx.x / 8) >= per || item >= nitem)
+    return;
+  const int sg = item / ntile, tile = item % ntile, split = sg / gsplit;
+  const int prod_begin = (sg % gsplit) * (NPROD / gsplit), prod_end = prod_begin + NPROD / gsplit;
+  const unsigned row_begin = (unsigned)split * rows_per_split;
+  const unsigned row_end = (row_begin + rows_per_split < nrows && split + 1 < nsplit) ? row_begin + rows_per_split : nrows;
+  acc += (size_t)split * NPROD * A3 * acc_stride;
+  const uint32_t tt = tile_list[tile];
+  const int ti = (int)(tt >> 16), tj = (int)(tt & 0xffffu);
+  const int li = threadIdx.x & 7, lj = threadIdx.x >> 3;
+  const int i0 = ti * 32 + li, j0 = tj * 32 + lj;
+  const int variant = (ti == tj ? 1 : 0) | (ti * 32 + 16 < N ? 0 : 2);
+  __shared__ __attribute__((aligned(16))) uint32_t sa[2 * UNITS * 4];
+  __shared__ __attribute__((aligned(16))) uint32_t sb[2 * UNITS * 4];
+  uint64_t cc[4][4], dd[4][4];
+#if defined(__HIP_DEVICE_COMPILE__)
+  constexpr bool DIRECT = true;
+#else
+  constexpr bool DIRECT = false;
+#endif
+  const size_t NS = fx_row_slots<FX>((size_t)N);
+  uint32_t va[DIRECT ? 1 : GL][4], vb[DIRECT ? 1 : GL][4];
+  uint32_t offa[GL], offb[GL];
+#pragma unroll
+  for(int g = 0; g < GL; ++g)
+    {
+      const int e = threadIdx.x + g * SYRK5_WG;
+      const int unit = e % 8, rr = e / 8;
+      offa[g] = (uint32_t)((size_t)rr * NS + ti * 32 + 4 * unit);
+      offb[g] = (uint32_t)((size_t)rr * NS + tj * 32 + 4 * unit);
+    }
+  auto fetch = [&](int plane, unsigned r0, int into) __attribute__((always_inline)) {
+    const uint32_t *base = fx + (size_t)plane * fx_stride + (size_t)r0 * NS;
+#pragma unroll
+    for(int g = 0; g < GL; ++g)
+      {
+        if constexpr(DIRECT)
+          {
+#if defined(__HIP_DEVICE_COMPILE__)
+            const int wbase = (into * UNITS + g * SYRK5_WG) * 4;
+            __builtin_amdgcn_global_load_lds((const __attribute__((address_space(1))) void *)(base + offa[g]),
+                                             (__attribute__((address_space(3))) void *)(sa + wbase), 16, 0, 0);
+            __builtin_amdgcn_global_load_lds((const __attribute__((address_space(1))) void *)(base + offb[g]),
+                                             (__attribute__((address_space(3))) void *)(sb + wbase), 16, 0, 0);
+#endif
+          }
+        else
+          {
+#pragma unroll
+            for(int l = 0; l < 4; ++l)
+              {
+                va[g][l] = base[offa[g] + l];
+                vb[g][l] = base[offb[g] + l];
+              }
+          }
+      }
+  };
+  auto store = [&](int buf) __attribute__((always_inline)) {
+    if constexpr(!DIRECT)
+      {
+#pragma unroll
+        for(int g = 0; g < GL; ++g)
+          {
+            const int e = threadIdx.x + g * SYRK5_WG;
+            piece_store<4>(sa + (buf * UNITS + e) * 4, va[g]);
+            piece_store<4>(sb + (buf * UNITS + e) * 4, vb[g]);
+          }
+      }
+  };
+  auto landed = [&]() __attribute__((always_inline)) {
+#if defined(__HIP_DEVICE_COMPILE__)
+    asm volatile("s_waitcnt vmcnt(0)" ::: "memory");
+#else
+    __syncthreads();
+#endif
+  };
+  auto rows = [&](auto variant_c, int buf) __attribute__((always_inline)) {
+    constexpr int V = decltype(variant_c)::value;
+    constexpr int PN = (V & 2) ? 2 : 4;
+    constexpr bool DIAG = (V & 1) != 0;
+#if defined(__HIP_DEVICE_COMPILE__)
+    typedef uint32_t u32x4 __attribute__((ext_vector_type(4)));
+    const uint32_t xa = (uint32_t)(uintptr_t)(__attribute__((address_space(3))) uint32_t *)(sa + buf * UNITS * 4 + li * 4);
+    const uint32_t xb = (uint32_t)(uintptr_t)(__attribute__((address_space(3))) uint32_t *)(sb + buf * UNITS * 4 + lj * 4);
+#define K2_L(C, A, B) "v_mad_u64_u32 %" #C ", vcc, %" #A ", %" #B ", %" #C "\n\t"
+#define K2_FULL                                                                                                                            \
+  K2_L(0, 16, 20) K2_L(1, 16, 21) K2_L(2, 16, 22) K2_L(3, 16, 23) K2_L(4, 17, 20) K2_L(5, 17, 21) K2_L(6, 17, 22) K2_L(7, 17, 23)          \
+  K2_L(8, 18, 20) K2_L(9, 18, 21) K2_L(10, 18, 22) K2_L(11, 18, 23) K2_L(12, 19, 20) K2_L(13, 19, 21) K2_L(14, 19, 22) K2_L(15, 19, 23)
+#define K2_DIAG                                                                                                                            \
+  K2_L(0, 16, 20) K2_L(4, 17, 20) K2_L(5, 17, 21) K2_L(8, 18, 20) K2_L(9, 18, 21) K2_L(10, 18, 22) K2_L(12, 19, 20) K2_L(13, 19, 21)       \
+  K2_L(14, 19, 22) K2_L(15, 19, 23)
+#define K2_HALF K2_L(0, 16, 20) K2_L(1, 16, 21) K2_L(2, 16, 22) K2_L(3, 16, 23) K2_L(4, 17, 20) K2_L(5, 17, 21) K2_L(6, 17, 22) K2_L(7, 17, 23)
+#define K2_HALF_DIAG K2_L(0, 16, 20) K2_L(4, 17, 20) K2_L(5, 17, 21)
+#define K2_MACS(va, vb)                                                                                                                    \
+  if constexpr(V == 0)                                                                                                                     \
+    {                                                                                                                                      \
+      K2_ASM(K2_FULL, va, vb)                                                                                                              \
+    }                                                                                                                                      \
+  else if constexpr(V == 1)                                                                                                                \
+    {                                                                                                                                      \
+      K2_ASM(K2_DIAG, va, vb)                                                                                                              \
+    }                                                                                                                                      \
+  else if constexpr(V == 2)                                                                                                                \
+    {                                                                                                                                      \
+      K2_ASM(K2_HALF, va, vb)                                                                                                              \
+    }                                                                                                                                      \
+  else                                                                                                                                     \
+    {                                                                                                                                      \
+      K2_ASM(K2_HALF_DIAG, va, vb)                                                                                                         \
+    }
+#define K2_ASM(MACS, va, vb)                                                                                                               \
+  asm volatile(MACS                                                                                                                        \
+               : "+v"(cc[0][0]), "+v"(cc[0][1]), "+v"(cc[0][2]), "+v"(cc[0][3]), "+v"(cc[1][0]), "+v"(cc[1][1]), "+v"(cc[1][2]),           \
+                 "+v"(cc[1][3]), "+v"(cc[2][0]), "+v"(cc[2][1]), "+v"(cc[2][2]), "+v"(cc[2][3]), "+v"(cc[3][0]), "+v"(cc[3][1]),           \
+                 "+v"(cc[3][2]), "+v"(cc[3][3])                                                                                            \
+               : "v"(va.x), "v"(va.y), "v"(va.z), "v"(va.w), "v"(vb.x), "v"(vb.y), "v"(vb.z), "v"(vb.w)                                    \
+               : "vcc");
+#define K2_NEXT(wa, wb, ra, rb, ROW)                                                                                                       \
+  asm volatile("s_waitcnt lgkmcnt(0)\n\tds_read_b128 %2, %4 offset:%6\n\tds_read_b128 %3, %5 offset:%6"                                   \
+               : "+v"(wa), "+v"(wb), "=&v"(ra), "=&v"(rb)                                                                                  \
+               : "v"(xa), "v"(xb), "n"((ROW) * 128)                                                                                        \
+               : "memory");
+#define K2_ROWS2(R) K2_NEXT(a0, b0, a1, b1, (R) + 1) K2_MACS(a0, b0) K2_NEXT(a1, b1, a0, b0, (R) + 2) K2_MACS(a1, b1)
+#define K2_ROWS8(R) K2_ROWS2(R) K2_ROWS2((R) + 2) K2_ROWS2((R) + 4) K2_ROWS2((R) + 6)
+    u32x4 a0, b0, a1, b1;
+    asm volatile("ds_read_b128 %0, %2\n\tds_read_b128 %1, %3" : "=&v"(a0), "=&v"(b0) : "v"(xa), "v"(xb) : "memory");
+    K2_ROWS8(0)
+    if constexpr(RBG == 32)
+      {
+        K2_ROWS8(8)
+        K2_ROWS8(16)
+      }
+    K2_ROWS2(RBG - 8)
+    K2_ROWS2(RBG - 6)
+    K2_ROWS2(RBG - 4)
+    K2_NEXT(a0, b0, a1, b1, RBG - 1)
+    K2_MACS(a0, b0)
+    asm volatile("s_waitcnt lgkmcnt(0)" : "+v"(a1), "+v"(b1)::"memory");
+    K2_MACS(a1, b1)
+#undef K2_ROWS8
+#undef K2_ROWS2
+#undef K2_NEXT
+#undef K2_ASM
+#undef K2_MACS
+#undef K2_HALF_DIAG
+#undef K2_HALF
+#undef K2_DIAG
+#undef K2_FULL
+#undef K2_L
+#else
+    const uint32_t *pa = sa + buf * UNITS * 4 + li * 4, *pb = sb + buf * UNITS * 4 + lj * 4;
+    for(int rr = 0; rr < RBG; ++rr)
+      {
+        uint32_t a[4], b[4];
+        piece_load<4>(pa + rr * 32, a);
+        piece_load<4>(pb + rr * 32, b);
+        syrk5k2_mac_row<PN, DIAG>(cc, a, b);
+      }
+#endif
+  };
+  for(int prod = prod_begin; prod < prod_end; ++prod)
+    for(int t = 0; t < 3; ++t)
+      {
+        const int plane = 3 * prod + t;
+#pragma unroll
+        for(int p = 0; p < 4; ++p)
+#pragma unroll
+          for(int q = 0; q < 4; ++q)
+            cc[p][q] = dd[p][q] = 0;
+        unsigned since = 0;
+        landed();
+        fetch(plane, row_begin, 0);
+        store(0);
+        landed();
+        auto sweep = [&](auto variant_c) __attribute__((always_inline)) {
+          int buf = 0;
+          for(unsigned r0 = row_begin; r0 < row_end; r0 += RBG)
+            {
+              fetch(plane, r0 + RBG < row_end ? r0 + RBG : row_begin, buf ^ 1);
+              rows(variant_c, buf);
+              syrk5k2_pass_end<RBG>(t, since, cc, dd);
+              store(buf ^ 1);
+              landed();
+              buf ^= 1;
+            }
+        };
+        switch(variant)
+          {
+          case 0: sweep(std::integral_constant<int, 0>()); break;
+          case 1: sweep(std::integral_constant<int, 1>()); break;
+          case 2: sweep(std::integral_constant<int, 2>()); break;
+          default: sweep(std::integral_constant<int, 3>()); break;
+          }
+#pragma unroll
+        for(int p = 0; p < 4; ++p)
+#pragma unroll
+          for(int q = 0; q < 4; ++q)
+            {
+              const int i = i0 + 8 * p, j = j0 + 8 * q;
+              if(i >= N || j > i)
+                continue;
+              uint32_t *o = acc + (size_t)(prod * A3) * acc_stride + (size_t)tile * 1024 + (size_t)(li + 8 * p) + (size_t)(lj + 8 * q) * 32;
+              unsigned __int128 v = syrk5k2_term(t, cc[p][q], dd[p][q]);
+              if(t > 0)
+                v += (unsigned __int128)o[0] | ((unsigned __int128)o[acc_stride] << 32) | ((unsigned __int128)o[2 * acc_stride] << 64)
+                     | ((unsigned __int128)o[3 * acc_stride] << 96);
+              else
+                o[4 * acc_stride] = 0;
+              o[0] = (uint32_t)v;
+              o[acc_stride] = (uint32_t)(v >> 32);
+              o[2 * acc_stride] = (uint32_t)(v >> 64);
+              o[3 * acc_stride] = (uint32_t)(v >> 96);
+            }
+      }
 }
 
 template <int FX>
@@ -3607,12 +3762,12 @@
 constexpr int T5_Z = 10;
 MW_HD void toom5_value(const uint32_t *fx, size_t fx_stride, int point, size_t e, uint32_t (&w)[4])
 {
-  const PiecePair lo = *reinterpret_cast<const PiecePair *>(fx + ((size_t)(3 * point + 0) * fx_stride + e) * 2);
-  const PiecePair hi = *reinterpret_cast<const PiecePair *>(fx + ((size_t)(3 * point + 1) * fx_stride + e) * 2);
-  w[0] = lo.w[0] | (lo.w[1] << 28);
-  w[1] = (lo.w[1] >> 4) | (hi.w[0] << 23);
-  w[2] = (hi.w[0] >> 9) | (hi.w[1] << 19);
-  w[3] = hi.w[1] >> 13;
+  const uint32_t lo0 = fx[(size_t)(9 * point + 0) * fx_stride + e], lo1 = fx[(size_t)(9 * point + 1) * fx_stride + e];
+  const uint32_t hi0 = fx[(size_t)(9 * point + 3) * fx_stride + e], hi1 = fx[(size_t)(9 * point + 4) * fx_stride + e];
+  w[0] = lo0 | (lo1 << 28);
+  w[1] = (lo1 >> 4) | (hi0 << 23);
+  w[2] = (hi0 >> 9) | (hi1 << 19);
+  w[3] = hi1 >> 13;
 }
 template <int FX>
 __global__ void __launch_bounds__(WG) k_fx_colsum5(const uint32_t *fx, size_t fx_stride, unsigned nrows, int N, unsigned rows_per_slice, uint32_t *partial)
diff --git a/sdpb_amd/csrc/solver.hpp b/sdpb_amd/csrc/solver.hpp
--- a/sdpb_amd/csrc/solver.hpp
+++ b/sdpb_amd/csrc/solver.hpp
@@ -810,7 +810,7 @@
     ss << (first ? "" : ", ") << "\"kernel.k_syrk_fx.ms\": " << syrk_kernel_ms_ << ", \"kernel.k_syrk_fx.launches\": " << syrk_launches_
        << ", \"kernel.k_syrk_fx.algorithmic_bytes\": " << (fx_bytes + acc_bytes)
        << ", \"kernel.k_syrk_fx.limb_macs\": "
-       << (double)Ptot_ * N_ * (N_ + 1) / 2 * FX * FX * (Syrk::SYRK_TOOM5K ? 27.0 / 64 : Syrk::SYRK_TOOM4K ? 21.0 / 64 : Syrk::SYRK_TOOM4 ? 7.0 / 16 : Syrk::SYRK_TWO_LEVEL ? 9.0 / 16 : 0.75)
+       << (double)Ptot_ * N_ * (N_ + 1) / 2 * FX * FX * (Syrk::SYRK_TOOM5K ? 81.0 / 256 : Syrk::SYRK_TOOM4K ? 21.0 / 64 : Syrk::SYRK_TOOM4 ? 7.0 / 16 : Syrk::SYRK_TWO_LEVEL ? 9.0 / 16 : 0.75)
        << ", \"kernel.k_syrk_fx.karatsuba_levels\": " << (Syrk::SYRK_TOOM4 ? 0 : Syrk::SYRK_TWO_LEVEL ? 2 : 1) << ", \"kernel.k_syrk_fx.toom4\": " << (Syrk::SYRK_TOOM4 ? 1 : 0) << ", \"kernel.k_syrk_fx.toom4k\": " << (Syrk::SYRK_TOOM4K ? 1 : 0) << ", \"kernel.k_syrk_fx.toom5k_lazy_carries\": " << (Syrk::SYRK_TOOM5K ? 1 : 0)
        << ", \"host_syncs\": " << host_syncs_ << ", \"launches\": " << launches_
        << ", \"iterations\": " << iteration_ << ", \"comm.world\": " << world_ << ", \"comm.ranks\": " << (comm_ ? comm_->ranks() : (world_ == 1 ? 1 : 0))
diff --git a/sdpb_amd/csrc/syrk_stage.hpp b/sdpb_amd/csrc/syrk_stage.hpp
--- a/sdpb_amd/csrc/syrk_stage.hpp
+++ b/sdpb_amd/csrc/syrk_stage.hpp
@@ -101,6 +101,8 @@
 #endif
   static constexpr int SYRK_RB = SYRK_TWO_LEVEL ? SDPB_SYRK2_RBG : (FX <= 24 ? 16 : 8);
   static constexpr size_t TILE_WORDS = (size_t)SYRK_PART_PLANES * SYRK_EDGE * SYRK_EDGE;
+  static constexpr int SYRK5_ROWS = SDPB_SYRK5_ROWS;
+  static_assert(!SYRK_TOOM5K || SYRK_RB % SYRK5_ROWS == 0, "a split begins and the image ends at whole passes of k_syrk5_k2");
 
   explicit FxSyrk(int num_cus) : num_cus_(num_cus), rec_(&own_) {}
   explicit FxSyrk(const FxSyrk *solver_stage) : num_cus_(solver_stage->num_cus_), rec_(solver_stage->rec_) {}
@@ -147,7 +149,7 @@
   }
   int syrk_splits_for(int tiles, unsigned nrows, size_t budget_words) const
   {
-    const int slots = num_cus_ * syrk_waves_per_simd<FX>();
+    const int slots = num_cus_ * (SYRK_TOOM5K ? syrk5_wg_per_cu(SYRK5_ROWS) : syrk_waves_per_simd<FX>());
     int nsplit = syrk_row_splits(tiles * syrk_group_split(), nrows, slots, SYRK_RB, SYRK_SPLIT_ROWS);
     const size_t per_split = TILE_WORDS * tiles;
     if(budget_words && (size_t)nsplit * per_split > budget_words)
@@ -357,7 +359,10 @@
         const dim3 grid(8 * cdiv((size_t)nt * nsplit, 8)), finish_grid(cdiv(total, WG));
         if constexpr(SYRK_TOOM4)
           {
-            if constexpr(SYRK_TOOM4K)
+            if constexpr(SYRK_TOOM5K)
+              launch(k_syrk5_k2<FX, SYRK5_ROWS>, dim3(8 * cdiv((size_t)nt * nsplit * gsplit, 8)), dim3(SYRK5_WG), stream, fx, win.stride, nrows, N, out,
+                     os, tl, nt, nsplit, rps, gsplit);
+            else if constexpr(SYRK_TOOM4K)
               launch(k_syrk_fx3<FX, SYRK_RB>, dim3(8 * cdiv((size_t)nt * nsplit * gsplit, 8)), dim3(WG), stream, fx, win.stride, nrows, N, out, os, tl,
                      nt, nsplit, rps, gsplit);
             else
diff --git a/sdpb_amd/workmodel.py b/sdpb_amd/workmodel.py
--- a/sdpb_amd/workmodel.py
+++ b/sdpb_amd/workmodel.py
@@ -66,10 +66,10 @@
     toom4k = fx in (16, 24, 32)
     toom5k = fx == 16
     two = fx % 4 == 0
-    words = 54 if toom5k else 21 * (fx // 8) if toom4k else 7 * (fx // 4) if toom4 else 9 * (fx // 4) if two else 3 * (fx // 2)
+    words = 81 if toom5k else 21 * (fx // 8) if toom4k else 7 * (fx // 4) if toom4 else 9 * (fx // 4) if two else 3 * (fx // 2)
     planes = 135 if toom5k else 21 * (2 * (fx // 8) + 1) if toom4k else 7 * (2 * (fx // 4) + 1) if toom4 else 2 * fx + 2
     rb = (16 if fx >= 32 else 32) if two else (16 if fx <= 24 else 8)
-    waves = 3 if toom4k else (3 if fx <= 16 else 2)
+    waves = 16 if toom5k else 3 if toom4k else (3 if fx <= 16 else 2)
     return fx, words, 32 if toom4k else 16, planes, rb, waves, toom4, toom4k
 
 
@@ -159,7 +159,7 @@
     ntile = tiles * (tiles + 1) // 2
 
     def planes_unbounded(r):
-        ns = syrk_row_splits(ntile * (21 if toom4k else 1), r, num_cus * waves, rb, 2560 if toom4k else 0) if r else 1
+        ns = syrk_row_splits(ntile * ((27 if fx == 16 else 21) if toom4k else 1), r, num_cus * waves, rb, 2560 if toom4k else 0) if r else 1
         return ns * planes * ntile * edge * edge * 4 if (ns > 1 or toom4) else 0
     unbounded = planes_unbounded(chunk_rows)
     budget = max(window - min(image, window // 2), 4)
```

New measurement: 6.656 (median of 6 runs). 5.0% higher.
